# deadskull7/One-Stop-for-COVID-19-Infection-and-Lung-Segmentation-plus-Classification

Measured on AMD Instinct MI355X. Metric: CT images/sec (fwd+bwd) U-Net 512x512x1 bs16, higher is better.
Workload: dtype f32 storage / accumulate / parameters; conv products as a two-term fp16 split (3 fp16 MFMAs per multiply, ~2^-22 per product; --algo 2 = strict fp32); 1 GPU; U-Net infection seg (task1 graph T1:853-916), 512x512x1, batch 16/GPU, fp32, fwd+loss+bwd+Keras-Adam; BASELINE.json configs[1]; storage=fp32, global_batch=16, parallelism=dp1, deterministic=False, bn_fold=2

## Files before the change

include/unet_hip.h:

```cpp
#ifndef UNET_HIP_H
#define UNET_HIP_H
#include <stddef.h>
#include <stdint.h>

#ifdef __cplusplus
extern "C" {
#endif

#define UNET_ABI_VERSION 16

typedef struct unet_ctx unet_ctx;
typedef struct unet_model unet_model;
typedef uint16_t unet_bf16;
enum { UNET_DTYPE_F32 = 0, UNET_DTYPE_BF16 = 1 };

enum { UNET_OK = 0, UNET_E_ARG = -1, UNET_E_HIP = -2, UNET_E_SHAPE = -3, UNET_E_STATE = -4, UNET_E_NODEV = -5 };

enum { UNET_ALGO_AUTO = 0, UNET_ALGO_NAIVE = 1, UNET_ALGO_MFMA = 2 };

int32_t unet_abi_version(void);
int32_t unet_ctx_create(int32_t device_id, unet_ctx** out);
void unet_ctx_destroy(unet_ctx* ctx);
const char* unet_last_error(const unet_ctx* ctx);
int32_t unet_ctx_set_profiling(unet_ctx* ctx, int32_t on);
enum { UNET_OPT_RELU_BITS = 1, UNET_OPT_BN_FOLD = 2, UNET_OPT_ENC_BN_FUSED = 3, UNET_OPT_BN_CONCAT_ANALYTIC = 4, UNET_OPT_BN_FUSE_STATS = 5, UNET_OPT_DETERMINISTIC = 6,
       UNET_OPT_HEAD_FUSED = 7, UNET_OPT_SKIP_RAW = 8, UNET_OPT_POOL_SUMS_FUSED = 9, UNET_OPT_HEAD_BWD_FUSED = 10, UNET_OPT_CONV_PP = 13, UNET_OPT_ENC_TAIL_DGRAD = 14 };
int32_t unet_ctx_set_option(unet_ctx* ctx, int32_t option, int32_t value);
int32_t unet_ctx_get_option(unet_ctx* ctx, int32_t option);

enum { UNET_ACT_NONE = 0, UNET_ACT_RELU = 1, UNET_ACT_ELU = 2 };
enum { UNET_MASK_NONE = 0, UNET_MASK_RELU = 1, UNET_MASK_ELU = 2, UNET_MASK_ELU_DROP = 3, UNET_MASK_RELU_BITS = 9  };

size_t unet_conv3x3_w_ws_floats(int32_t cin, int32_t cout);
int32_t unet_conv3x3_pick_algo(int32_t algo, int32_t wd, int32_t cin, int32_t cout);
double unet_conv3x3_exec_ratio(int32_t algo, int32_t h, int32_t wd, int32_t cin, int32_t cout);
double unet_conv3x3_wgrad_exec_ratio(int32_t algo, int32_t h, int32_t wd, int32_t cin, int32_t cout);
int32_t unet_request_bn_stats(unet_ctx*, int32_t c);
int32_t unet_relu_bits_supported(int32_t algo, int32_t h, int32_t wd, int32_t cin, int32_t cout);
size_t unet_relu_bits_bytes(int32_t n, int32_t h, int32_t wd, int32_t c);
int32_t unet_request_relu_bits(unet_ctx*, void* bits);
int32_t unet_allow_k_slices(unet_ctx*);
int32_t unet_ctx_max_kernel_scratch_bytes(unet_ctx*);
int32_t unet_conv3x3_fwd(unet_ctx*, const float* x, const float* w, const float* bias, float* y,
                         int32_t n, int32_t h, int32_t wd, int32_t cin, int32_t cout,
                         int32_t act, float drop_rate, uint64_t drop_seed, int32_t algo, float* w_ws, void* stream);
int32_t unet_conv3x3_fwd_ld(unet_ctx*, const float* x, const float* w, const float* bias, float* y, int32_t ldy,
                            int32_t n, int32_t h, int32_t wd, int32_t cin, int32_t cout, int32_t act, int32_t algo, float* w_ws, void* stream);
int32_t unet_conv3x3_bwd_data(unet_ctx*, const float* dy, const float* w, const float* mask_src,
                              int32_t mask_mode, float mask_rate, uint64_t mask_seed,
                              float* dx, float* wt_ws, int32_t n, int32_t h, int32_t wd,
                              int32_t cin, int32_t cout, int32_t algo, void* stream);
int32_t unet_conv3x3_bnfold_supported(int32_t algo, int32_t h, int32_t wd, int32_t cin, int32_t cout);
size_t unet_conv3x3_bnfold_ws_floats(int32_t n, int32_t cin, int32_t cout);
int32_t unet_conv3x3_bnfold_fwd(unet_ctx*, const float* x, const float* bnp, const float* w, const float* bias, float* y, int32_t n, int32_t h,
                                int32_t wd, int32_t cin, int32_t cout, int32_t act, int32_t algo, float* ws, void* stream);
int32_t unet_conv3x3_bnfold_bwd_weights(unet_ctx*, const float* x, const float* bnp, const float* dy, const float* w, float* dw, float* db,
                                        double* bn_bwd_sums, void* gws, size_t gws_bytes, float* ws, int32_t n, int32_t h, int32_t wd,
                                        int32_t cin, int32_t cout, int32_t algo, void* stream);
int32_t unet_conv3x3_bnfold_bwd_data(unet_ctx*, const float* dy, const float* w, const float* bnp, const double* bn_bwd_sums, double count, const float* x,
                                     int32_t x_channels, int32_t mask_mode, float mask_rate, uint64_t mask_seed, float* dx, float* wt_ws, float* coef,
                                     int32_t n, int32_t h, int32_t wd, int32_t cin, int32_t cout, int32_t algo, void* stream);
int32_t unet_conv3x3_bnfold_bwd_data_enc_tail(unet_ctx*, const float* dy, const float* w, const float* bnp, const double* bn_bwd_sums, double count, const float* x, int32_t ldx,
                                              const float* enc_bnp, const double* enc_sums, double enc_count, const float* skip_k1, const float* dy_pooled, float rate,
                                              uint64_t seed, float* dx, float* wt_ws, float* coef, int32_t n, int32_t h, int32_t wd, int32_t c, int32_t algo, void* stream);
size_t unet_conv3x3_bwd_weights_ws_bytes(int32_t n, int32_t h, int32_t wd, int32_t cin, int32_t cout);
int32_t unet_conv3x3_bwd_weights(unet_ctx*, const float* x, const float* dy, float* dw, float* db,
                                 void* ws, size_t ws_bytes, int32_t n, int32_t h, int32_t wd,
                                 int32_t cin, int32_t cout, int32_t algo, void* stream);

int32_t unet_convT2x2_fwd(unet_ctx*, const float* x, const float* w, const float* bias, float* y,
                          int32_t ldy, int32_t n, int32_t h, int32_t wd, int32_t cin, int32_t cout,
                          int32_t algo, void* stream);
int32_t unet_convT2x2_bwd_data(unet_ctx*, const float* dy, int32_t lddy, const float* w,
                               const float* relu_src, float* dx, int32_t n, int32_t h, int32_t wd,
                               int32_t cin, int32_t cout, int32_t algo, void* stream);
size_t unet_convT2x2_bwd_weights_ws_bytes(int32_t n, int32_t h, int32_t wd, int32_t cin, int32_t cout);
int32_t unet_convT2x2_bwd_weights(unet_ctx*, const float* x, const float* dy, int32_t lddy,
                                  float* dw, float* db, void* ws, size_t ws_bytes, int32_t n,
                                  int32_t h, int32_t wd, int32_t cin, int32_t cout, int32_t algo,
                                  void* stream);

int32_t unet_bn_stats(unet_ctx*, const float* x, int32_t ldx, double* sums, int64_t pixels,
                      int32_t c, void* stream);
int32_t unet_bn_stats_concat(unet_ctx*, const float* x_up, int32_t ldx, const double* src_sums, double src_count, const float* src_gamma,
                             const float* src_beta, double* sums, int64_t pixels, int32_t c_up, int32_t c_skip, void* stream);
int32_t unet_bn_finalize_train(unet_ctx*, const double* sums, double count, const float* gamma,
                               const float* beta, float* moving_mean, float* moving_var,
                               float* bnp, int32_t c, void* stream);
int32_t unet_bn_finalize_infer(unet_ctx*, const float* gamma, const float* beta,
                               const float* moving_mean, const float* moving_var, float* bnp,
                               int32_t c, void* stream);
int32_t unet_bn_apply(unet_ctx*, const float* x, int32_t ldx, const float* bnp, float* y,
                      int32_t ldy, int64_t pixels, int32_t c, void* stream);
int32_t unet_bn_bwd_stats(unet_ctx*, const float* dy, int32_t lddy, const float* x, int32_t ldx,
                          const float* bnp, double* sums, int64_t pixels, int32_t c, void* stream);
int32_t unet_bn_bwd_param_grads(unet_ctx*, const double* sums, float* dgamma, float* dbeta,
                                int32_t c, void* stream);
int32_t unet_bn_bwd_apply(unet_ctx*, const float* dy, int32_t lddy, const float* x, int32_t ldx,
                          const float* bnp, const double* sums, double count, int32_t mask_mode,
                          float mask_rate, uint64_t mask_seed, float* dx, int32_t lddx, int64_t pixels,
                          int32_t c, void* stream);

int32_t unet_maxpool2x2_dropout_fwd(unet_ctx*, const float* x, int32_t ldx, float* y, int32_t n,
                                    int32_t h, int32_t wd, int32_t c, float rate, uint64_t seed,
                                    void* stream);
int32_t unet_maxpool2x2_dropout_bwd(unet_ctx*, const float* x, int32_t ldx, const float* dy,
                                    float* dx, int32_t lddx, int32_t n, int32_t h, int32_t wd,
                                    int32_t c, float rate, uint64_t seed, int32_t accumulate,
                                    void* stream);

int32_t unet_bn_apply_maxpool_dropout_fwd(unet_ctx*, const float* x, int32_t ldx, const float* bnp, float* y,
                                          int32_t ldy, float* pooled, int32_t n, int32_t h, int32_t wd,
                                          int32_t c, float rate, uint64_t seed, void* stream);
int32_t unet_maxpool2x2_dropout_bwd_bnstats(unet_ctx*, const float* y, int32_t ldy, const float* dy, float* dx,
                                            int32_t lddx, const float* gamma, const float* beta, double* sums,
                                            int32_t n, int32_t h, int32_t wd, int32_t c, float rate,
                                            uint64_t seed, void* stream);
// ... 371 lines not shown
```

one-stop-for-covid-19-infection-and-lung-segmentation-plus-classification_amd/_lib.py:

```python
from __future__ import annotations

import ctypes as C
import os

_HERE = os.path.dirname(os.path.abspath(__file__))
LIB_PATH = os.environ.get("COVIDSEG_AMD_LIB") or os.path.join(_HERE, "libunet_hip.so")
ABI_VERSION = 16
COMM_HANDLE_BYTES, COMM_MAX_WORLD, COMM_MAX_DOUBLES = 64, 8, 2048

ALGO_AUTO, ALGO_NAIVE, ALGO_MFMA = 0, 1, 2
OPTIONS = {"relu_bits": 1, "bn_fold": 2, "enc_bn_fused": 3, "bn_concat_analytic": 4, "bn_fuse_stats": 5, "deterministic": 6, "head_fused": 7, "skip_raw": 8, "pool_sums_fused": 9, "head_bwd_fused": 10, "conv_pp": 13, "enc_tail_dgrad": 14}
ARCH_UNET, ARCH_UNETPP, ARCH_CLASSIFIER = 0, 1, 2
LOSSES = {"bce_dice_loss": 0, "binary_crossentropy": 1, "dice_loss": 2, "tversky_loss": 3, "weighted_bce_dice_loss": 4}
DTYPE_F32, DTYPE_BF16 = 0, 1
ACT_NONE, ACT_RELU, ACT_ELU = 0, 1, 2
MORPH_OPS = {"dilate": 0, "erode": 1, "open": 2, "close": 3}
MORPH_MAX_ITERATIONS = 64
INTENSITY_MAX_EDGES = 63
JOINT_HIST_MAX_K, JOINT_HIST_MAX_BINS = 16, 64
SMOOTH_MAX_RADIUS = 32
PAIRS_CHUNK, PAIRS_LDS_SLOTS = 4096, 1024
PAIRS_MIN_CAPACITY, PAIRS_MAX_CAPACITY = 16, 2 ** 30
TRACK_CLS_NONE, TRACK_CLS_RESOLVED, TRACK_CLS_SHRINKAGE, TRACK_CLS_BOTH, TRACK_CLS_GROWTH, TRACK_CLS_NEW = 0, 1, 2, 3, 4, 5
TEXTURE_MAX_LEVELS, TEXTURE_MAX_DISTANCE, TEXTURE_LDS_COUNTERS = 64, 4, 8192
TEXTURE_MAX_RUN = 2 ** 15
ZONE_MAX_PARTS, ZONE_MAX_SHELLS, ZONE_MAX_BINS = 8, 4, 1024
MASK_NONE, MASK_RELU, MASK_ELU, MASK_ELU_DROP = 0, 1, 2, 3
PROG_FWD_TRAIN, PROG_BWD, PROG_FWD_INFER = 0, 1, 2
SYNC_BN_FWD, SYNC_LOSS, SYNC_BN_BWD, SYNC_GRAD_BUCKET = 0, 1, 2, 3

f32p = C.POINTER(C.c_float)
f64p = C.POINTER(C.c_double)
vp = C.c_void_p
i32, i64, u64, f32, f64, sz = C.c_int32, C.c_int64, C.c_uint64, C.c_float, C.c_double, C.c_size_t


class SyncPoint(C.Structure):
    _fields_ = [("after_op", i32), ("kind", i32), ("ptr", vp), ("count", i64), ("use_op", i32), ("reserved", i32)]


RENDER_MAX_TILES, RENDER_MAX_LAYERS = 64, 4


class RenderTile(C.Structure):
    _fields_ = [("axis", i32), ("index", i32), ("x0", i32), ("y0", i32), ("w", i32), ("h", i32)]


class RenderLayer(C.Structure):
    _fields_ = [("labels", vp), ("palette", vp), ("dtype", i32), ("palette_size", i32), ("fill_alpha", i32), ("outline_alpha", i32)]


class ZoneSpec(C.Structure):
    _fields_ = [("parts", i32 * 3), ("flip", i32 * 3), ("lo", (i32 * 3) * 2), ("extent", (i32 * 3) * 2), ("shells", i32), ("reserved", i32), ("r2", (f64 * 3) * 2)]


_PROTOS = {
    "unet_abi_version": (i32, []),
    "unet_ctx_create": (i32, [i32, C.POINTER(vp)]),
    "unet_ctx_destroy": (None, [vp]),
    "unet_last_error": (C.c_char_p, [vp]),
    "unet_ctx_set_profiling": (i32, [vp, i32]),
    "unet_ctx_set_option": (i32, [vp, i32, i32]),
    "unet_ctx_get_option": (i32, [vp, i32]),
    "unet_conv3x3_w_ws_floats": (sz, [i32, i32]),
    "unet_conv3x3_pick_algo": (i32, [i32, i32, i32, i32]),
    "unet_conv3x3_exec_ratio": (f64, [i32, i32, i32, i32, i32]),
    "unet_conv3x3_wgrad_exec_ratio": (f64, [i32, i32, i32, i32, i32]),
    "unet_request_bn_stats": (i32, [vp, i32]),
    "unet_relu_bits_supported": (i32, [i32, i32, i32, i32, i32]),
    "unet_relu_bits_bytes": (sz, [i32, i32, i32, i32]),
    "unet_request_relu_bits": (i32, [vp, vp]),
    "unet_allow_k_slices": (i32, [vp]),
    "unet_ctx_max_kernel_scratch_bytes": (i32, [vp]),
    "unet_conv3x3_fwd": (i32, [vp, vp, vp, vp, vp, i32, i32, i32, i32, i32, i32, f32, u64, i32, vp, vp]),
    "unet_conv3x3_fwd_ld": (i32, [vp, vp, vp, vp, vp, i32, i32, i32, i32, i32, i32, i32, i32, vp, vp]),
    "unet_conv3x3_bwd_data": (i32, [vp, vp, vp, vp, i32, f32, u64, vp, vp, i32, i32, i32, i32, i32, i32, vp]),
    "unet_conv3x3_bwd_weights_ws_bytes": (sz, [i32, i32, i32, i32, i32]),
    "unet_conv3x3_bwd_weights": (i32, [vp, vp, vp, vp, vp, vp, sz, i32, i32, i32, i32, i32, i32, vp]),
    "unet_convT2x2_fwd": (i32, [vp, vp, vp, vp, vp, i32, i32, i32, i32, i32, i32, i32, vp]),
    "unet_convT2x2_bwd_data": (i32, [vp, vp, i32, vp, vp, vp, i32, i32, i32, i32, i32, i32, vp]),
    "unet_convT2x2_bwd_weights_ws_bytes": (sz, [i32, i32, i32, i32, i32]),
    "unet_convT2x2_bwd_weights": (i32, [vp, vp, vp, i32, vp, vp, vp, sz, i32, i32, i32, i32, i32, i32, vp]),
    "unet_cast_f32_to_bf16": (i32, [vp, vp, vp, i64, vp]),
    "unet_cast_bf16_to_f32": (i32, [vp, vp, vp, i64, vp]),
    "unet_conv3x3_fwd_bf16": (i32, [vp, vp, vp, vp, vp, i32, i32, i32, i32, i32, i32, f32, u64, vp, vp]),
    "unet_conv3x3_first_fwd_bf16": (i32, [vp, vp, vp, vp, vp, i32, i32, i32, i32, i32, f32, u64, vp]),
    "unet_conv3x3_bwd_data_bf16": (i32, [vp, vp, vp, vp, i32, f32, u64, vp, vp, i32, i32, i32, i32, i32, vp]),
    "unet_conv3x3_bwd_weights_ws_bytes_bf16": (sz, [i32, i32, i32, i32, i32]),
    "unet_conv3x3_bwd_weights_bf16": (i32, [vp, vp, vp, vp, vp, vp, sz, i32, i32, i32, i32, i32, vp]),
    "unet_conv3x3_first_bwd_weights_bf16": (i32, [vp, vp, vp, vp, vp, vp, sz, i32, i32, i32, i32, vp]),
    "unet_convT2x2_fwd_bf16": (i32, [vp, vp, vp, vp, vp, i32, i32, i32, i32, i32, i32, vp, vp]),
    "unet_convT2x2_bwd_data_bf16": (i32, [vp, vp, i32, vp, vp, vp, i32, i32, i32, i32, i32, vp, vp]),
    "unet_convT2x2_bwd_weights_ws_bytes_bf16": (sz, [i32, i32, i32, i32, i32]),
    "unet_convT2x2_bwd_weights_bf16": (i32, [vp, vp, vp, i32, vp, vp, vp, sz, i32, i32, i32, i32, i32, vp]),
    "unet_bn_stats": (i32, [vp, vp, i32, vp, i64, i32, vp]),
    "unet_bn_stats_bf16": (i32, [vp, vp, i32, vp, i64, i32, vp]),
    "unet_conv3x3_bnfold_supported": (i32, [i32, i32, i32, i32, i32]),
    "unet_conv3x3_bnfold_ws_floats": (sz, [i32, i32, i32]),
    "unet_conv3x3_bnfold_fwd": (i32, [vp, vp, vp, vp, vp, vp, i32, i32, i32, i32, i32, i32, i32, vp, vp]),
    "unet_conv3x3_bnfold_bwd_weights": (i32, [vp, vp, vp, vp, vp, vp, vp, vp, vp, sz, vp, i32, i32, i32, i32, i32, i32, vp]),
    "unet_conv3x3_bnfold_bwd_data": (i32, [vp, vp, vp, vp, vp, f64, vp, i32, i32, f32, u64, vp, vp, vp, i32, i32, i32, i32, i32, i32, vp]),
    "unet_conv3x3_bnfold_bwd_data_enc_tail": (i32, [vp, vp, vp, vp, vp, f64, vp, i32, vp, vp, f64, vp, vp, f32, u64, vp, vp, vp, i32, i32, i32, i32, i32, vp]),
    "unet_bn_stats_concat": (i32, [vp, vp, i32, vp, f64, vp, vp, vp, i64, i32, i32, vp]),
    "unet_bn_stats_concat_bf16": (i32, [vp, vp, i32, vp, f64, vp, vp, vp, i64, i32, i32, vp]),
    "unet_bn_finalize_train": (i32, [vp, vp, f64, vp, vp, vp, vp, vp, i32, vp]),
    "unet_bn_finalize_infer": (i32, [vp, vp, vp, vp, vp, vp, i32, vp]),
    "unet_bn_apply": (i32, [vp, vp, i32, vp, vp, i32, i64, i32, vp]),
    "unet_bn_apply_bf16": (i32, [vp, vp, i32, vp, vp, i32, i64, i32, vp]),
    "unet_bn_bwd_stats": (i32, [vp, vp, i32, vp, i32, vp, vp, i64, i32, vp]),
    "unet_bn_bwd_stats_bf16": (i32, [vp, vp, i32, vp, i32, vp, vp, i64, i32, vp]),
    "unet_bn_bwd_param_grads": (i32, [vp, vp, vp, vp, i32, vp]),
    "unet_bn_bwd_apply": (i32, [vp, vp, i32, vp, i32, vp, vp, f64, i32, f32, u64, vp, i32, i64, i32, vp]),
    "unet_bn_bwd_apply_bf16": (i32, [vp, vp, i32, vp, i32, vp, vp, f64, i32, f32, u64, vp, i32, i64, i32, vp]),
    "unet_maxpool2x2_dropout_fwd": (i32, [vp, vp, i32, vp, i32, i32, i32, i32, f32, u64, vp]),
    "unet_maxpool2x2_dropout_fwd_bf16": (i32, [vp, vp, i32, vp, i32, i32, i32, i32, f32, u64, vp]),
    "unet_maxpool2x2_dropout_bwd": (i32, [vp, vp, i32, vp, vp, i32, i32, i32, i32, i32, f32, u64, i32, vp]),
    "unet_maxpool2x2_dropout_bwd_bf16": (i32, [vp, vp, i32, vp, vp, i32, i32, i32, i32, i32, f32, u64, i32, vp]),
    "unet_bn_apply_maxpool_dropout_fwd": (i32, [vp, vp, i32, vp, vp, i32, vp, i32, i32, i32, i32, f32, u64, vp]),
    "unet_bn_apply_maxpool_dropout_fwd_bf16": (i32, [vp, vp, i32, vp, vp, i32, vp, i32, i32, i32, i32, f32, u64, vp]),
    "unet_maxpool2x2_dropout_bwd_bnstats": (i32, [vp, vp, i32, vp, vp, i32, vp, vp, vp, i32, i32, i32, i32, f32, u64, vp]),
    "unet_maxpool2x2_dropout_bwd_sums": (i32, [vp, vp, vp, vp, vp, vp, i32, i32, i32, i32, f32, u64, vp]),
    "unet_maxpool2x2_dropout_bwd_sums_bf16": (i32, [vp, vp, vp, vp, vp, vp, i32, i32, i32, i32, f32, u64, vp]),
    "unet_bn_maxpool_bwd_apply_bf16": (i32, [vp, vp, i32, vp, vp, f64, vp, i32, vp, vp, i32, i32, i32, i32, i32, f32, u64, vp]),
    "unet_bn_bwd_skip_term": (i32, [vp, vp, vp, vp, vp, vp, i32, f64, vp]),
    "unet_bn_maxpool_bwd_apply": (i32, [vp, vp, i32, vp, vp, f64, vp, i32, vp, vp, i32, i32, i32, i32, i32, f32, u64, vp]),
    "unet_maxpool2x2_dropout_bwd_bnstats_bf16": (i32, [vp, vp, i32, vp, vp, i32, vp, vp, vp, i32, i32, i32, i32, f32, u64, vp]),
    "unet_head_fwd": (i32, [vp, vp, vp, vp, vp, vp, vp, i64, i32, vp]),
    "unet_head_fwd_bf16": (i32, [vp, vp, vp, vp, vp, vp, vp, i64, i32, vp]),
    "unet_loss_finalize": (i32, [vp, vp, f64, vp, vp]),
    "unet_head_bwd": (i32, [vp, vp, vp, vp, vp, vp, f64, vp, vp, vp, i64, i32, i32, vp]),
    "unet_head_bwd_bf16": (i32, [vp, vp, vp, vp, vp, vp, f64, vp, vp, vp, i64, i32, i32, vp]),
    "unet_loss_finalize_ex": (i32, [vp, vp, f64, i32, f32, f32, vp, vp]),
    "unet_head_bwd_ex": (i32, [vp, vp, vp, vp, vp, vp, f64, i32, f32, f32, vp, vp, vp, vp, i64, i32, i32, vp]),
    "unet_head_bwd_bf16_ex": (i32, [vp, vp, vp, vp, vp, vp, f64, i32, f32, f32, vp, vp, vp, vp, i64, i32, i32, vp]),
    "unet_head_fwd_ex": (i32, [vp, vp, vp, vp, vp, vp, vp, vp, i64, i32, vp]),
    "unet_head_fwd_bf16_ex": (i32, [vp, vp, vp, vp, vp, vp, vp, vp, i64, i32, vp]),
    "unet_loss_weight_map": (i32, [vp, vp, vp, i32, i32, i32, vp]),
    "unet_conv3x3_head_fwd_ex": (i32, [vp, vp, vp, vp, vp, vp, vp, vp, vp, vp, vp, vp, i32, i32, i32, i32, vp, vp]),
    "unet_adam_keras": (i32, [vp, vp, vp, vp, vp, i64, f32, f32, f32, f32, f32, vp]),
    "unet_seg_metrics_sweep": (i32, [vp, vp, vp, vp, i32, vp, i64, vp]),
    "unet_gather_samples": (i32, [vp, vp, vp, vp, i64, i64, vp]),
    "unet_augment_samples": (i32, [vp, vp, vp, vp, vp, vp, vp, i64, i32, i32, i32, vp]),
    "unet_feat_col_mean": (i32, [vp, vp, i64, i64, i64, vp, vp]),
    "unet_feat_gemm_nt_workspace": (sz, [i64, i64, i64, i32]),
    "unet_feat_gemm_nt": (i32, [vp, vp, i64, vp, vp, i64, vp, i64, i64, i64, i32, vp, i64, i32, vp, sz, vp]),
    "unet_feat_gemm_tn_workspace": (sz, [i64, i64, i64]),
    "unet_feat_gemm_tn": (i32, [vp, vp, i64, vp, i64, vp, i64, i64, i64, vp, i64, i32, vp, sz, vp]),
    "unet_kmeans_step": (i32, [vp, vp, i64, i64, i64, vp, i32, vp, vp, vp, vp, vp, vp]),
    "unet_cluster_route_workspace": (sz, [i64, i64, i32]),
    "unet_cluster_route": (i32, [vp, vp, i32, i64, i32, i32, i32, i64, vp, vp, i32, vp, i32, vp, vp, vp, vp, sz, vp]),
    "unet_conv3x3_head_supported": (i32, [vp, i32, i32, i32, i32]),
    "unet_conv3x3_head_fwd": (i32, [vp, vp, vp, vp, vp, vp, vp, vp, vp, vp, vp, i32, i32, i32, i32, vp, vp]),
    "unet_conv3x3_bwd_data_pool_sums_supported": (i32, [vp, i32, i32, i32, i32]),
    "unet_conv3x3_bwd_data_pool_sums": (i32, [vp, vp, vp, vp, vp, vp, f32, vp, vp, vp, i32, i32, i32, i32, i32, vp]),
    "unet_head_dy": (i32, [vp, vp, vp, vp, f64, vp, vp, vp, vp, vp, vp, vp, i32, i32, i32, vp]),
# ... 195 lines not shown
```

one-stop-for-covid-19-infection-and-lung-segmentation-plus-classification_amd/csrc/common.h:

```cpp
#pragma once
#include <hip/hip_runtime.h>
#include <stdint.h>
#include <stdio.h>
#include <set>
#include <string>

#include "../../include/unet_hip.h"

constexpr int UNET_BN_SLOTS = 64, UNET_BN_SLOTS_DET = 1024, UNET_BN_SLOT_DOUBLES = 2048;
struct unet_loss_sel { int32_t kind = UNET_LOSS_BCE_DICE; float alpha = 0.5f, beta = 0.5f; };
inline bool unet_loss_sel_ok(const unet_loss_sel& ls, const float* wm = nullptr, bool need_map = true) {
  if (ls.kind < UNET_LOSS_BCE_DICE || ls.kind > UNET_LOSS_WEIGHTED_BCE_DICE) return false;
  if (ls.kind == UNET_LOSS_TVERSKY && !(ls.alpha > 0.0f && ls.beta > 0.0f && ls.alpha < 1e30f && ls.beta < 1e30f)) return false;
  return !need_map || (ls.kind == UNET_LOSS_WEIGHTED_BCE_DICE) == (wm != nullptr);
}
constexpr int UNET_HEAD_SUMS = 100;
struct unet_ctx {
  int device = 0;
  int num_cu = 256;
  int profiling = 0;
  int opt_relu_bits = 1;
  int opt_bn_fold = 2;
  int opt_enc_bn_fused = 1;
  int opt_bn_concat_analytic = 1;
  int opt_bn_fuse_stats = 1;
  int opt_pool_sums_fused = 1;
  int opt_skip_raw = 1;
  int opt_head_fused = 1;
  int opt_head_bwd_fused = 1;
  int opt_enc_tail_dgrad = 1;
  int opt_conv_pp = 1;
  int opt_deterministic = 0;
  double* bn_slots = nullptr;
  int bn_nslots() const { return opt_deterministic ? UNET_BN_SLOTS_DET : UNET_BN_SLOTS; }
  void* convt_img = nullptr;
  size_t convt_img_bytes = 0;
  int k_slices_ok = 0;
  void* splitk_ws = nullptr;
  size_t splitk_ws_bytes = 0;
  int stats_req_c = 0;
  const void* stats_in_slots = nullptr;
  int stats_in_slots_c = 0;
  bool stats_in_slots_xs = false;
  unsigned long long* signs_req = nullptr;
  const void* signs_done = nullptr;
  std::set<const void*> big_lds_kernels;
  std::set<const void*> noted_kernels;
  int max_scratch_bytes = 0;
  std::string err;
};

#define UNET_FAIL(ctx, code, ...)                         \
  do {                                                    \
    char _b[512];                                         \
    snprintf(_b, sizeof(_b), __VA_ARGS__);                \
    if (ctx) (ctx)->err = _b;                             \
    return (code);                                        \
  } while (0)

#define UNET_CHECK_LAUNCH(ctx, what)                                              \
  do {                                                                            \
    hipError_t _e = hipGetLastError();                                            \
    if (_e != hipSuccess) UNET_FAIL(ctx, UNET_E_HIP, "%s: %s", what, hipGetErrorString(_e)); \
  } while (0)

#define UNET_HIP(ctx, expr)                                                       \
  do {                                                                            \
    hipError_t _e = (expr);                                                       \
    if (_e != hipSuccess) UNET_FAIL(ctx, UNET_E_HIP, "%s: %s", #expr, hipGetErrorString(_e)); \
  } while (0)

static inline int32_t unet_big_lds(unet_ctx* ctx, const void* kernel, size_t bytes, const char* what) {
  if (ctx->big_lds_kernels.count(kernel)) return UNET_OK;
  if (hipFuncSetAttribute(kernel, hipFuncAttributeMaxDynamicSharedMemorySize, (int)bytes) != hipSuccess) UNET_FAIL(ctx, UNET_E_HIP, "%s: cannot reserve %zu bytes of LDS", what, bytes);
  ctx->big_lds_kernels.insert(kernel);
  return UNET_OK;
}
static inline void unet_note_kernel(unet_ctx* ctx, const void* kernel) {
  if (ctx->noted_kernels.count(kernel)) return;
  ctx->noted_kernels.insert(kernel);
  hipFuncAttributes at;
  if (hipFuncGetAttributes(&at, kernel) == hipSuccess && (int)at.localSizeBytes > ctx->max_scratch_bytes) ctx->max_scratch_bytes = (int)at.localSizeBytes;
}
// ... 143 lines not shown
}

enum { ACT_NONE = 0, ACT_RELU = 1, ACT_ELU = 2 };
__device__ __forceinline__ float apply_act(float v, int act) {
  if (act == ACT_RELU) return fmaxf(v, 0.0f);
  if (act == ACT_ELU) return v > 0.0f ? v : expm1f(v);
  return v;
}
enum { MASK_NONE = 0, MASK_RELU = 1, MASK_ELU = 2, MASK_ELU_DROP = 3 };
enum { MASK_BIAS_TAB = 4 };
enum { MASK_BN_BWD = 5 };
enum { MASK_BN_BWD_ELU = 6, MASK_BN_BWD_ELU_DROP = 7 };
enum { MASK_BN_BWD_RELU = 8 };
enum { MASK_RELU_BITS = 9 };
enum { MASK_POOL_SUMS = 10 };
int32_t k_bn_bwd_coef(unet_ctx*, const float* bnp, const double* sums, double count, float* coef, int c, hipStream_t s);
__device__ __forceinline__ float mask_factor(float m, int mode, float ks , float rate) {
  if (mode == MASK_RELU) return m > 0.0f ? 1.0f : 0.0f;
  if (mode == MASK_ELU) return m > 0.0f ? 1.0f : m + 1.0f;
  if (mode == MASK_ELU_DROP) { const float a = m * (1.0f - rate); return ks * (a > 0.0f ? 1.0f : a + 1.0f); }
  return 1.0f;
}

size_t bn_fold_scratch_floats(int cin, int cout);
int32_t k_bn_fold_prepare(unet_ctx*, const float* w, const float* bias, const float* scale, const float* shift, int cin, int cout, float* scratch, hipStream_t s, bool want_scaled = true);
size_t wgrad_bn_fold_scratch_floats(int n, int cout);
bool wgrad_bn_fold_supported(int cout);
int32_t k_wgrad_bn_fold_fix(unet_ctx*, const float* dy, int n, int h, int wd, int cin, int cout, const float* scale, const float* shift, float* dw, const float* db, float* scratch,
                            hipStream_t s, const float* w = nullptr, const float* mean = nullptr, const float* istd = nullptr, double* bn_bwd_sums = nullptr,
                            const float* pre_s = nullptr, const float* pre_t = nullptr,
                            float* dgamma = nullptr, float* dbeta = nullptr);
int32_t k_wgrad_bn_fold_fix_bf16(unet_ctx*, const unet_bf16* dy, int n, int h, int wd, int cin, int cout, const float* scale, const float* shift, float* dw, const float* db,
                                 float* scratch, hipStream_t s, const float* w = nullptr, const float* mean = nullptr, const float* istd = nullptr, double* bn_bwd_sums = nullptr);
constexpr int UNET_PREP_MAX = 36;
bool h2_conv3x3_selected(int algo, int K, int M);
bool pp_conv3x3_selected(const unet_ctx* ctx, int K, int M, int n, int h, int wd, const float* mask, int mask_mode, int act, float rate, int ldy);
int32_t k_conv3x3_pp_fwd(unet_ctx*, const float* x, const void* wimg, const float* bias, const float* mask, int mask_mode, float* y, int ldy, int n, int h, int wd, int K, int M,
                         int act, hipStream_t s, bool vdy = false);
size_t h2_wimg_bytes(int K, int M);
int32_t k_h2_weights(unet_ctx*, const float* w, void* img, int cin, int cout, int flip, hipStream_t s, const float* cs = nullptr);
int32_t k_h2_weights_multi(unet_ctx*, const float* const* w, void* const* img, const int* cin, const int* cout, const int* flip, int count, hipStream_t s);
int32_t k_h2_weights_bound(unet_ctx*, const float* w, const float* cs, void* img, int cin, int cout, hipStream_t s);
int32_t k_h2_prep_multi(unet_ctx*, const float* const* w, const float* const* cs, void* const* img, const int* cin, const int* cout, const int* kind, int count, hipStream_t s);
size_t h2_convT_img_bytes(int cin, int cout);
int32_t k_conv3x3_h2_fwd(unet_ctx*, const float* x, const void* wimg, const float* bias, const float* mask, int mask_mode, float* y, int n, int h, int wd, int K, int M,
                         int act, float rate, uint64_t seed, hipStream_t s, int mask_climit = 1 << 30, int ldy = 0);
int32_t k_slot_fold(unet_ctx*, double* sums, int count, hipStream_t s, bool xs = false);
int32_t k_enc_tail_finish(unet_ctx*, double* sums, const double* dec_sum_dyxhat, const float* dec_invstd, const float* dec_gamma, const float* gamma, float* dgamma, float* dbeta, int c,
                          double frac, hipStream_t s);
bool h2_enc_tail_dgrad_selected(const unet_ctx* ctx, int algo, int n, int h, int wd, int C, bool force);
int32_t k_conv3x3_h2_dgrad_bn_bwd_up(unet_ctx*, const float* dy, const void* wimg, const float* coef, const float* x, float* dx, int n, int h, int wd, int C, hipStream_t s);
int32_t k_conv3x3_h2_dgrad_enc_tail(unet_ctx*, const float* dy, const void* wimg, const float* coef, const float* x, int ldx, const float* enc_bnp, const double* enc_sums, double count,
                                    const float* skip_k1, const float* dy_pooled, float* dx, int n, int h, int wd, int C, float rate, uint64_t seed, hipStream_t s);
bool h2_pool_sums_selected(const unet_ctx* ctx, int algo, int wd, int K, int M);
int32_t k_conv3x3_h2_dgrad_pool_sums(unet_ctx*, const float* dy, const void* wimg, const float* pooled, const float* gamma, const float* beta, float rate, float* dx, double* sums,
                                     int n, int h, int wd, int K, int M, hipStream_t s);
int32_t k_bn_finalize_compose(unet_ctx*, int training, const double* sums, double count, const float* gamma, const float* beta, float* mm, float* mv, float* bnp, int c,
                              const float* enc_bnp, float* comp, hipStream_t s);
int32_t k_loss_finalize(unet_ctx*, const double* loss_sums, double count, float* loss_out, float* loss_out2, hipStream_t s, unet_loss_sel ls = {});
int32_t k_cls_loss_finalize(unet_ctx*, const double* sums, double count, float* out, float* out2, hipStream_t s);
int32_t k_bn_compose(unet_ctx*, const float* bnp_dec, const float* bnp_enc, float* comp, int c, hipStream_t s);
struct h2_head_args { const float* w = nullptr; const float* b = nullptr; float* p = nullptr; const float* t = nullptr; double* slots = nullptr; float aux = 0.0f; const float* wm = nullptr; double inv_count = 0.0; };
bool h2_conv3x3_head_selected(const unet_ctx* ctx, int algo, int wd, int K, int M);
int32_t k_conv3x3_h2_head_fwd(unet_ctx*, const float* x, const void* wimg, const float* bias, float* y, const float* wh, const float* bh, float* p, const float* t,
                              int n, int h, int wd, int K, hipStream_t s, const float* wm = nullptr);
int32_t k_head_fold(unet_ctx*, double* loss_sums, double* head_sums, hipStream_t s, bool weighted = false);
int32_t k_loss_weight_map(unet_ctx*, const float* y_true, float* weight, int n, int h, int wd, hipStream_t s);
int32_t k_head_dy(unet_ctx*, const float* p, const float* t, const double* loss_sums, double count, const double* head_sums, const float* w, const unsigned long long* bits,
                  const float* y, float* dy, float* dw, float* db, int n, int h, int wd, hipStream_t s, unet_loss_sel ls = {}, const float* wm = nullptr);
int32_t k_bn_maxpool_bwd_apply_k1(unet_ctx*, const float* x, int ldx, const float* bnp, const double* sums, double count, const float* g_skip, int ldg, const float* skip_k1,
                                  const float* dy_pooled, float* dx, int lddx, int n, int h, int wd, int c, float rate, uint64_t seed, hipStream_t s);
bool h2_convT_selected(const unet_ctx* ctx, int algo, int cin, int cout);
int32_t k_convT_h2_fwd(unet_ctx*, const float* x, const float* w, const float* bias, float* y, int ldy, int n, int h, int wd, int cin, int cout, hipStream_t s, const void* prepared = nullptr);
int32_t k_convT_h2_dgrad(unet_ctx*, const float* dy, int lddy, const float* w, const float* mask, float* dx, int n, int h, int wd, int cin, int cout, hipStream_t s, int mask_bits = 0,
                         const void* prepared = nullptr);
bool h2_wgrad_selected(int algo, int cin, int cout);
bool h2_wgrad_c16_selected(int algo, int wd, int cin, int cout);
size_t h2_wgrad_c16_ws_bytes(int n, int h, int wd);
int32_t k_wgrad_c16_gather(unet_ctx*, const float* G, float* dw, float* db, hipStream_t s);
int32_t k_conv3x3_h2_wgrad_c16(unet_ctx*, const float* x, const float* dy, float* dw, float* db, void* ws, size_t ws_bytes, int n, int h, int wd, hipStream_t s);
size_t h2_wgrad_ws_bytes(int n, int h, int wd, int cin, int cout);
int32_t k_conv3x3_h2_wgrad(unet_ctx*, const float* x, const float* dy, float* dw, float* db, void* ws, size_t ws_bytes, int n, int h, int wd, int cin, int cout, hipStream_t s);
int32_t k_head_dzm(unet_ctx*, const float* p, const float* t, const double* loss_sums, double count, const double* head_sums, const unsigned long long* bits, void* dzm, float* dw,
                   float* db, int n, int h, int wd, hipStream_t s, unet_loss_sel ls = {}, const float* wm = nullptr);
bool h2_head_bwd_selected(const unet_ctx* ctx, int algo, int wd, int cin);
int32_t k_conv3x3_h2_dgrad_dzm(unet_ctx*, const void* dzm, const void* wimg, const float* mask, int mask_mode, float* dx, int n, int h, int wd, int M, hipStream_t s);
int32_t k_conv3x3_h2_wgrad_dzm(unet_ctx*, const float* x, const void* dzm, const float* w_head, float* dw, float* db, void* ws, size_t ws_bytes, int n, int h, int wd, int cin,
                               hipStream_t s);
int32_t k_conv3x3_naive_fwd(unet_ctx*, const float* x, const float* w, const float* bias, const float* mask, int mask_mode,
                            float* y, int n, int h, int wd, int cin, int cout, int act, float rate, uint64_t seed, hipStream_t s);
bool c1_relu_bits_supported(int wd, int cout);
int32_t k_conv3x3_c1_fwd_bits(unet_ctx*, const float* x, const float* w, const float* bias, float* y, unsigned long long* signs, int n, int h, int wd, int cout, hipStream_t s);
int32_t k_conv3x3_c1_fwd(unet_ctx*, const float* x, const float* w, const float* bias, float* y, int n, int h,
                         int wd, int cout, int act, float rate, uint64_t seed, hipStream_t s);
size_t c1_wgrad_ws_bytes(int cout);
int32_t k_conv3x3_c1_wgrad(unet_ctx*, const float* x, const float* dy, float* dw, float* db, void* ws, size_t ws_bytes, int n, int h,
                           int wd, int cout, hipStream_t s);
int32_t k_flip_transpose_w3x3(unet_ctx*, const float* w, float* wt, int cin, int cout, hipStream_t s);
int32_t k_conv3x3_naive_wgrad(unet_ctx*, const float* x, const float* dy, float* dw, float* db, int n, int h,
                              int wd, int cin, int cout, hipStream_t s);
int32_t k_convT_naive_fwd(unet_ctx*, const float* x, const float* w, const float* bias, float* y, int ldy, int n,
                          int h, int wd, int cin, int cout, hipStream_t s);
int32_t k_convT_naive_dgrad(unet_ctx*, const float* dy, int lddy, const float* w, const float* mask, float* dx,
                            int n, int h, int wd, int cin, int cout, hipStream_t s);
int32_t k_convT_naive_wgrad(unet_ctx*, const float* x, const float* dy, int lddy, float* dw, float* db, int n,
                            int h, int wd, int cin, int cout, hipStream_t s);
// ... 47 lines not shown
```

one-stop-for-covid-19-infection-and-lung-segmentation-plus-classification_amd/csrc/kernels_conv_h2.hip:

```cpp
#include <stdlib.h>

#include <algorithm>

#include "common.h"

#ifndef H2_EXPERIMENT
#define H2_EXPERIMENT 0
#endif

#if H2_EXPERIMENT == 5
__device__ unsigned long long h2_trace[16384 * 16];
#define H2_STAMP(i) do { if (tid == 0 && blockIdx.x < 16384) h2_trace[blockIdx.x * 16 + (i)] = __builtin_readcyclecounter(); } while (0)
extern "C" int32_t unet_debug_h2_trace(unsigned long long* host, int n) {
  return hipMemcpyFromSymbol(host, HIP_SYMBOL(h2_trace), (size_t)n * 8) == hipSuccess ? 0 : 1;
}
#else
#define H2_STAMP(i) do { } while (0)
#endif
namespace {

typedef _Float16 f16x8 __attribute__((ext_vector_type(8)));
typedef _Float16 f16x2 __attribute__((ext_vector_type(2)));
typedef unet_f32x16 f32x16;
constexpr int H2_HEADER = 256;
// ... 48 lines not shown
#pragma unroll
  for (int o = 32; o >= 1; o >>= 1) mx = fmaxf(mx, __shfl_xor(mx, o));
  if (p.cs_bound) {
    float mc = 0.f;
    for (int i = threadIdx.x & 63; i < p.cs_mod; i += 64) mc = fmaxf(mc, fabsf(p.cs[i]));
#pragma unroll
    for (int o = 32; o >= 1; o >>= 1) mc = fmaxf(mc, __shfl_xor(mc, o));
    mx *= mc;
  }
  const int eb = (int)((__float_as_uint(mx) >> 23) & 0xFF);
  int e = eb >= 11 ? scale_exp_for(eb) : 0;
  e = min(max(e, -100), 100);
  const float sc = pow2f(e);
  if (blockIdx.x == 0 && threadIdx.x == 0) { hdr[0] = pow2f(-e); hdr[1] = sc; }
  unet_bf16* const img = p.img + H2_HEADER / 2;
  for (long long el = (long long)blockIdx.x * 256 + threadIdx.x; el < p.total; el += (long long)gridDim.x * 256) {
    long long r = el;
    const int m = (int)(r & 31); r >>= 5;
    const int half = (int)(r & 1); r >>= 1;
    const int nb = (int)(r % NB); r /= NB;
    const int tap = (int)(r % T); r /= T;
    const int ks = (int)(r % KS); r /= KS;
    const int chunk = (int)(r % nchunks); const int g = (int)(r / nchunks);
    const long long k0 = ((long long)chunk * KS + ks) * 16 + half * 8;
    const long long mm = ((long long)g * NB + nb) * 32 + cperm(m);
    const float* src = p.w + (long long)(p.flip ? T - 1 - tap : tap) * p.tap_stride + k0 * p.sk + mm * p.sm;
    unsigned hh[4], ml[4];
#pragma unroll
    for (int j = 0; j < 4; ++j) {
      float a = mm < M ? src[(2 * j) * p.sk] * sc : 0.0f, b = mm < M ? src[(2 * j + 1) * p.sk] * sc : 0.0f;
      if (p.cs) { a *= p.cs[k0 + 2 * j]; b *= p.cs[k0 + 2 * j + 1]; }
      split2(a, b, hh[j], ml[j]);
    }
    const long long base = ((((((long long)g * nchunks + chunk) * KS + ks) * T + tap) * NB + nb) * 2 * 2 + half) * 32 + m;
    *reinterpret_cast<uint4*>(img + (base + 0 * 64) * 8) = make_uint4(hh[0], hh[1], hh[2], hh[3]);
    *reinterpret_cast<uint4*>(img + (base + 1 * 64) * 8) = make_uint4(ml[0], ml[1], ml[2], ml[3]);
  }
}

__device__ __forceinline__ f16x8 lds_frag(const char* p) { return *reinterpret_cast<const f16x8*>(p); }
__device__ __forceinline__ int out_cell(int p, int c) { return p * 128 + ((c ^ (p & 7)) << 4); }

template <int MODE, int NB, int RW, bool GEN, int WPS, int EPI = 0, bool SPLITK = false>
__global__ __launch_bounds__(256, WPS) void conv_h2_kernel(const float* __restrict__ x, int ldx, const unet_bf16* __restrict__ wimg_hdr, const float* __restrict__ bias,
                                                           const float* __restrict__ mask, float* __restrict__ y, int ldy, int N, int H, int W, int K, int M, int act,
                                                           int mask_mode, float rate, unsigned long long seed, int tiles_x, int tiles_y, int groups,
                                                           int total_blocks, double* __restrict__ stats, int stats_c, unsigned long long* __restrict__ signs,
                                                           int mask_climit, h2_head_args hd, int img_nb, int xs, int kcps, long long y_split, int g0, int gtot, int ldm, int c_off) {
  constexpr bool HEAD = EPI == 1 || EPI == 4, WHEAD = EPI == 4, POOLS = EPI == 2;
  constexpr bool VDY = EPI == 3;
  constexpr bool ETAIL = EPI == 5;
  static_assert(!ETAIL || (MODE == 0 && RW == 2 && !GEN && !SPLITK), "the encoder-tail epilogue rides on the 8-row conv3x3 data-gradient launches");
  if (ETAIL) { mask_mode = MASK_BN_BWD; act = ACT_NONE; stats = nullptr; signs = nullptr; }
  static_assert(!VDY || (MODE == 0 && NB == 1 && RW == 2 && !GEN), "the virtual head gradient feeds the 32-channel data-gradient launch");
  static_assert(!HEAD || (MODE == 0 && NB == 1 && RW == 2 && !GEN), "the fused head rides on the 32-channel forward kernel");
  static_assert(!POOLS || (MODE == 0 && !GEN), "the pooled sums ride on a plain conv3x3 data-gradient launch");
  static_assert(!SPLITK || (MODE == 0 && EPI == 0 && !GEN), "K slices: plain conv3x3 launches");
  if (POOLS) { mask_mode = MASK_POOL_SUMS; act = ACT_NONE; signs = nullptr; }
  if (HEAD) { mask_mode = MASK_NONE; act = ACT_RELU; stats = nullptr; }
  constexpr int T = MODE == 0 ? 9 : 1, KS = MODE == 0 ? 1 : 2;
  constexpr int TH = 4 * RW;
  constexpr int PR = MODE == 0 ? TH + 2 : TH, PWD = MODE == 0 ? 34 : 32, NPIX = PR * PWD;
  constexpr int HS = NPIX * 16 + (MODE == 0 ? 0 : 64);
  constexpr int PLANE = KS * 2 * HS;
  constexpr int IN_BYTES = 2 * PLANE, W_BYTES = KS * T * NB * 2 * 2 * 32 * 16;
  constexpr int PPIECES = KS * NPIX * 4, WPIECES = W_BYTES / 16;
  constexpr int PL = (PPIECES + 255) / 256, WL = (WPIECES + 255) / 256;
  constexpr int OUT_PS = 128;
  constexpr bool WPAD = NB != 1 || MODE != 0;
  constexpr int W_LDS = WPAD ? WL * 256 * 16 : W_BYTES;
  extern __shared__ __attribute__((aligned(16))) char smem[];
  char* const s_in = smem; char* const s_w = smem + IN_BYTES;
  float* const s_amax = reinterpret_cast<float*>(smem + IN_BYTES + W_LDS);
  float* const s_bias = s_amax + 4;

  const int tid = threadIdx.x, lane = tid & 63, l31 = lane & 31, hi = lane >> 5;
  const int wave = __builtin_amdgcn_readfirstlane(tid >> 6);
  const int per = gridDim.x >> 3;
  const int wi = (blockIdx.x & 7) * per + (blockIdx.x >> 3);
  if (wi >= total_blocks) return;
  const int g = g0 + wi % groups; int t = wi / groups;
  const int tx = t % tiles_x; t /= tiles_x;
  const int ty = t % tiles_y; const int n = t / tiles_y;
  const int x0 = tx * 32, y0 = ty * TH;
  const int HI = MODE == 2 ? 2 * H : H, WI = MODE == 2 ? 2 * W : W;
  const int nchunks = K / (16 * KS);
  const int cbeg = SPLITK ? (int)blockIdx.y * kcps : 0, cend = SPLITK ? min(cbeg + kcps, nchunks) : nchunks;
  if (SPLITK) y += (long long)blockIdx.y * y_split;
  const unet_bf16* const wimg = wimg_hdr + H2_HEADER / 2;
  const float w_unscale = *reinterpret_cast<const float*>(wimg_hdr);

  f32x16 acc[RW][NB];
#pragma unroll
  for (int i = 0; i < RW; ++i)
#pragma unroll
    for (int j = 0; j < NB; ++j)
#pragma unroll
      for (int r = 0; r < 16; ++r) acc[i][j][r] = 0.0f;

  const __amdgpu_buffer_rsrc_t rs_x = make_rsrc(x + (long long)n * HI * WI * ldx, (long long)HI * WI * ldx * 4);
  const __amdgpu_buffer_rsrc_t rs_w = __builtin_amdgcn_make_buffer_rsrc(const_cast<unet_bf16*>(wimg), 0, (int)((long long)gtot * nchunks * W_BYTES), 0x00020000);
  int poff[PL];
#pragma unroll
  for (int k = 0; k < PL; ++k) {
    const int idx = tid + k * 256;
    const int q = idx & 3, pp = idx >> 2, ks = pp / NPIX, pix = pp - ks * NPIX;
// ... 375 lines not shown
        gp[q * 4] = g4.x; gp[q * 4 + 1] = g4.y; gp[q * 4 + 2] = g4.z; gp[q * 4 + 3] = g4.w;
      }
#pragma unroll
      for (int r = 0; r < RW; ++r)
#pragma unroll
        for (int j = 0; j < 4; ++j) *reinterpret_cast<float4*>(s_x + r * 4096 + out_cell(j * 8 + (lane >> 3), lane & 7)) = mpre[nb][r][j];
#pragma unroll
      for (int q = 0; q < 4; ++q) {
        const int cc = nb * 32 + hi * 16 + q * 4;
        const float4 xa4 = *reinterpret_cast<const float4*>(s_x + out_cell(l31, hi * 4 + q)), xb4 = *reinterpret_cast<const float4*>(s_x + 4096 + out_cell(l31, hi * 4 + q));
        const float4 c0 = *reinterpret_cast<const float4*>(s_bias + cc), ck = *reinterpret_cast<const float4*>(s_bias + NB * 32 + cc), c2 = *reinterpret_cast<const float4*>(s_bias + 2 * NB * 32 + cc);
        const float4 sc4 = *reinterpret_cast<const float4*>(s_co + cc), sh4 = *reinterpret_cast<const float4*>(s_co + NB * 32 + cc), mn4 = *reinterpret_cast<const float4*>(s_co + 2 * NB * 32 + cc);
        const float4 is4 = *reinterpret_cast<const float4*>(s_co + 3 * NB * 32 + cc), k14 = *reinterpret_cast<const float4*>(s_co + 4 * NB * 32 + cc), k24 = *reinterpret_cast<const float4*>(s_co + 5 * NB * 32 + cc);
        const float xa[4] = {xa4.x, xa4.y, xa4.z, xa4.w}, xb[4] = {xb4.x, xb4.y, xb4.z, xb4.w};
        const float K0[4] = {c0.x, c0.y, c0.z, c0.w}, kk[4] = {ck.x, ck.y, ck.z, ck.w}, K2[4] = {c2.x, c2.y, c2.z, c2.w}, sc[4] = {sc4.x, sc4.y, sc4.z, sc4.w}, sh[4] = {sh4.x, sh4.y, sh4.z, sh4.w};
        const float mean[4] = {mn4.x, mn4.y, mn4.z, mn4.w}, istd[4] = {is4.x, is4.y, is4.z, is4.w}, k1[4] = {k14.x, k14.y, k14.z, k14.w}, k2[4] = {k24.x, k24.y, k24.z, k24.w};
#pragma unroll
        for (int c = 0; c < 4; ++c) {
          const int i = q * 4 + c;
          const float gsa = fmaf(K0[c], acc[0][nb][i] * unscale, K2[c]), gsb = fmaf(K0[c], acc[1][nb][i] * unscale, K2[c]);
          const float ya = fmaf(xa[c], sc[c], sh[c]), yb = fmaf(xb[c], sc[c], sh[c]);
          const float pa = __int_as_float(__builtin_amdgcn_update_dpp(0, __float_as_int(ya), 0xB1, 0xF, 0xF, true));
          const float pb = __int_as_float(__builtin_amdgcn_update_dpp(0, __float_as_int(yb), 0xB1, 0xF, 0xF, true));
          const int kmax = argmax4(odd ? pa : ya, odd ? ya : pa, odd ? pb : yb, odd ? yb : pb);
          const float ta = fmaf(kk[c], ya, gsa) + (kmax == odd ? gp[i] : 0.f);
          const float tb = fmaf(kk[c], yb, gsb) + (kmax == 2 + odd ? gp[i] : 0.f);
          acc[0][nb][i] = xa[c] > 0.f ? sc[c] * (ta - k1[c] - (xa[c] - mean[c]) * istd[c] * k2[c]) : 0.f;
          acc[1][nb][i] = xb[c] > 0.f ? sc[c] * (tb - k1[c] - (xb[c] - mean[c]) * istd[c] * k2[c]) : 0.f;
        }
      }
#pragma unroll
      for (int r = 0; r < RW; ++r) {
        const int py = py0 + r;
#pragma unroll
        for (int q = 0; q < 4; ++q)
          *reinterpret_cast<float4*>(s_x + out_cell(l31, hi * 4 + q)) = make_float4(acc[r][nb][q * 4], acc[r][nb][q * 4 + 1], acc[r][nb][q * 4 + 2], acc[r][nb][q * 4 + 3]);
        float4 t4s[4];
#pragma unroll
        for (int j = 0; j < 4; ++j) t4s[j] = *reinterpret_cast<const float4*>(s_x + out_cell(j * 8 + (lane >> 3), lane & 7));
        asm volatile("" :: "v"(t4s[0].x), "v"(t4s[1].x), "v"(t4s[2].x), "v"(t4s[3].x));
#pragma unroll
        for (int j = 0; j < 4; ++j) {
          const int pxj = x0 + j * 8 + (lane >> 3), cj = lane & 7;
          if (pxj < W && mb0 + cj * 4 < M) {
            float* const q = y + (((long long)n * H + py) * W + pxj) * ldy + (mb0 - c_off) + cj * 4;
            __builtin_nontemporal_store(t4s[j].x, q); __builtin_nontemporal_store(t4s[j].y, q + 1); __builtin_nontemporal_store(t4s[j].z, q + 2); __builtin_nontemporal_store(t4s[j].w, q + 3);
          }
        }
      }
    }
    H2_STAMP(8);
    return;
  }
#pragma unroll
  for (int nb = 0; nb < NB; ++nb) {
    const int mb0 = (g * NB + nb) * 32, mb = mb0 + hi * 16;
    if (mb0 >= M) continue;
    int ab = 0, oc = mb;
    if (MODE == 1) { const int ct = M >> 2; ab = mb / ct; oc = mb - ab * ct; }
    float bv[16];
#pragma unroll
    for (int q = 0; q < 4; ++q) {
      const float4 b4 = *reinterpret_cast<const float4*>(s_bias + nb * 32 + hi * 16 + q * 4);
      bv[q * 4] = b4.x; bv[q * 4 + 1] = b4.y; bv[q * 4 + 2] = b4.z; bv[q * 4 + 3] = b4.w;
    }
    float4 st1 = make_float4(0.f, 0.f, 0.f, 0.f), st2 = st1;
#pragma unroll
    for (int r = 0; r < RW; ++r) {
      const int py = y0 + wave * RW + r;
      if (py >= H) continue;
      const bool live = px_ < W && mb < M;
      long long o;
      if (MODE == 1) o = (((long long)n * 2 * H + 2 * py + (ab >> 1)) * (2 * W) + 2 * px_ + (ab & 1)) * ldy + oc;
      else o = (((long long)n * H + py) * W + px_) * ldy + mb;
      float v[16], mv[16], a[16];
#pragma unroll
      for (int i = 0; i < 16; ++i) a[i] = acc[r][nb][i] * unscale;
      if (mask_mode == MASK_RELU_BITS) {
        float4 w01, w23;
        if (MPF) { w01 = mpre[MPF ? nb : 0][MPF ? r : 0][0]; w23 = mpre[MPF ? nb : 0][MPF ? r : 0][1]; }
        else {
          const bool ok = py < H && x0 + (l31 & ~7) < W;
          const unsigned long long* p = reinterpret_cast<const unsigned long long*>(mask) + ((((long long)n * H + py) * (W >> 3) + (x0 >> 3) + (l31 >> 3)) * (M >> 5) + (g * NB + nb)) * 4;
          w01 = ok ? *reinterpret_cast<const float4*>(p) : make_float4(0.f, 0.f, 0.f, 0.f);
          w23 = ok ? *reinterpret_cast<const float4*>(p + 2) : make_float4(0.f, 0.f, 0.f, 0.f);
        }
        const bool up = (l31 & 4) != 0;
        const unsigned d[4] = {__float_as_uint(up ? w01.y : w01.x), __float_as_uint(up ? w01.w : w01.z), __float_as_uint(up ? w23.y : w23.x), __float_as_uint(up ? w23.w : w23.z)};
        const int sh = (l31 & 3) * 8 + hi * 4;
#pragma unroll
        for (int q = 0; q < 4; ++q)
#pragma unroll
          for (int k = 0; k < 4; ++k) mv[q * 4 + k] = ((d[k] >> (sh + q)) & 1u) ? 1.0f : 0.0f;
      } else if (want_m && !POOLS) {
        if (MPF) {
#pragma unroll
          for (int j = 0; j < 4; ++j) *reinterpret_cast<float4*>(s_out + out_cell(j * 8 + (lane >> 3), lane & 7)) = mpre[MPF ? nb : 0][MPF ? r : 0][j];
        }
#pragma unroll
        for (int q = 0; q < 4; ++q) {
          float4 m4;
          if (MPF) m4 = *reinterpret_cast<const float4*>(s_out + out_cell(l31, hi * 4 + q));
          else m4 = (live && mb0 < mask_climit) ? *reinterpret_cast<const float4*>(mask + (((long long)n * H + py) * W + px_) * ldm + (mb - c_off) + q * 4) : make_float4(0.f, 0.f, 0.f, 0.f);
          mv[q * 4] = m4.x; mv[q * 4 + 1] = m4.y; mv[q * 4 + 2] = m4.z; mv[q * 4 + 3] = m4.w;
        }
      }
      if (mask_mode >= MASK_BN_BWD && mask_mode <= MASK_BN_BWD_RELU) {
#pragma unroll
        for (int q = 0; q < 4; ++q) {
          const float4 k1 = *reinterpret_cast<const float4*>(s_bias + (NB + nb) * 32 + hi * 16 + q * 4), k2 = *reinterpret_cast<const float4*>(s_bias + (2 * NB + nb) * 32 + hi * 16 + q * 4);
          v[q * 4] = fmaf(bv[q * 4], a[q * 4], fmaf(k1.x, mv[q * 4], k2.x));
          v[q * 4 + 1] = fmaf(bv[q * 4 + 1], a[q * 4 + 1], fmaf(k1.y, mv[q * 4 + 1], k2.y));
          v[q * 4 + 2] = fmaf(bv[q * 4 + 2], a[q * 4 + 2], fmaf(k1.z, mv[q * 4 + 2], k2.z));
          v[q * 4 + 3] = fmaf(bv[q * 4 + 3], a[q * 4 + 3], fmaf(k1.w, mv[q * 4 + 3], k2.w));
        }
        if (mask_mode == MASK_BN_BWD_RELU) {
#pragma unroll
          for (int i = 0; i < 16; ++i) v[i] = mv[i] > 0.f ? v[i] : 0.f;
        }
      } else if (mask_mode == MASK_BIAS_TAB && (py == 0 || py == H - 1 || px_ == 0 || px_ == W - 1)) {
        const int cls = (((py == 0) | ((py == H - 1) << 1)) << 2) | ((px_ == 0) | ((px_ == W - 1) << 1));
        const float* tb = mask + (long long)cls * M + mb;
#pragma unroll
        for (int q = 0; q < 4; ++q) {
          const float4 b4 = *reinterpret_cast<const float4*>(tb + q * 4);
          v[q * 4] = a[q * 4] + b4.x; v[q * 4 + 1] = a[q * 4 + 1] + b4.y; v[q * 4 + 2] = a[q * 4 + 2] + b4.z; v[q * 4 + 3] = a[q * 4 + 3] + b4.w;
        }
      } else {
#pragma unroll
        for (int i = 0; i < 16; ++i) v[i] = a[i] + bv[i];
      }
      if (!GEN) {
        if (act == ACT_RELU) {
#pragma unroll
          for (int i = 0; i < 16; ++i) v[i] = fmaxf(v[i], 0.f);
        }
        if (mask_mode == MASK_RELU || mask_mode == MASK_RELU_BITS) {
#pragma unroll
          for (int i = 0; i < 16; ++i) v[i] = mv[i] > 0.f ? v[i] : 0.f;
        }
      } else {
#pragma unroll
        for (int i = 0; i < 16; ++i) v[i] = apply_act(v[i], act);
        if (mask_mode >= MASK_BN_BWD && mask_mode <= MASK_BN_BWD_RELU) {
          if (mask_mode == MASK_BN_BWD_ELU || mask_mode == MASK_BN_BWD_ELU_DROP) {
            const int mm = mask_mode == MASK_BN_BWD_ELU_DROP ? MASK_ELU_DROP : MASK_ELU;
#pragma unroll
            for (int q = 0; q < 4; ++q) {
              float4 ks4 = make_float4(1.f, 1.f, 1.f, 1.f);
              if (mm == MASK_ELU_DROP) ks4 = keep_scale((o >> 2) + q, rate, seed);
              v[q * 4] *= mask_factor(mv[q * 4], mm, ks4.x, rate); v[q * 4 + 1] *= mask_factor(mv[q * 4 + 1], mm, ks4.y, rate);
              v[q * 4 + 2] *= mask_factor(mv[q * 4 + 2], mm, ks4.z, rate); v[q * 4 + 3] *= mask_factor(mv[q * 4 + 3], mm, ks4.w, rate);
            }
          }
        } else if (mask_mode == MASK_NONE || mask_mode == MASK_BIAS_TAB) {
          if (rate > 0.0f) {
#pragma unroll
            for (int q = 0; q < 4; ++q) {
              const float4 ks4 = keep_scale((o >> 2) + q, rate, seed);
              v[q * 4] *= ks4.x; v[q * 4 + 1] *= ks4.y; v[q * 4 + 2] *= ks4.z; v[q * 4 + 3] *= ks4.w;
            }
          }
        } else {
#pragma unroll
          for (int q = 0; q < 4; ++q) {
            float4 ks4 = make_float4(1.f, 1.f, 1.f, 1.f);
            if (mask_mode == MASK_ELU_DROP) ks4 = keep_scale((o >> 2) + q, rate, seed);
            v[q * 4] *= mask_factor(mv[q * 4], mask_mode, ks4.x, rate); v[q * 4 + 1] *= mask_factor(mv[q * 4 + 1], mask_mode, ks4.y, rate);
            v[q * 4 + 2] *= mask_factor(mv[q * 4 + 2], mask_mode, ks4.z, rate); v[q * 4 + 3] *= mask_factor(mv[q * 4 + 3], mask_mode, ks4.w, rate);
          }
        }
      }
#pragma unroll
      for (int q = 0; q < 4; ++q)
        *reinterpret_cast<float4*>(s_out + out_cell(l31, hi * 4 + q)) = make_float4(v[q * 4], v[q * 4 + 1], v[q * 4 + 2], v[q * 4 + 3]);
      float4 t4s[4];
      if (!GEN) {
#pragma unroll
        for (int j = 0; j < 4; ++j) t4s[j] = *reinterpret_cast<const float4*>(s_out + out_cell(j * 8 + (lane >> 3), lane & 7));
        asm volatile("" :: "v"(t4s[0].x), "v"(t4s[1].x), "v"(t4s[2].x), "v"(t4s[3].x));
      }
#pragma unroll
      for (int j = 0; j < 4; ++j) {
        const int pj = j * 8 + (lane >> 3), cj = lane & 7, pxj = x0 + pj;
        const float4 t4 = GEN ? *reinterpret_cast<const float4*>(s_out + out_cell(pj, cj)) : t4s[j];
        long long oj;
        if (MODE == 1) oj = (((long long)n * 2 * H + 2 * py + (ab >> 1)) * (2 * W) + 2 * pxj + (ab & 1)) * ldy + (oc - hi * 16);
        else oj = (((long long)n * H + py) * W + pxj) * ldy + (mb - hi * 16);
        if (MODE == 0 && !GEN && signs) {
          const unsigned long long bb[4] = {__builtin_amdgcn_ballot_w64(t4.x > 0.f), __builtin_amdgcn_ballot_w64(t4.y > 0.f), __builtin_amdgcn_ballot_w64(t4.z > 0.f), __builtin_amdgcn_ballot_w64(t4.w > 0.f)};
          int slo = 0, shi = 0;
          unet_writelane(slo, (unsigned)bb[0], 0); unet_writelane(shi, (unsigned)(bb[0] >> 32), 0); unet_writelane(slo, (unsigned)bb[1], 1); unet_writelane(shi, (unsigned)(bb[1] >> 32), 1);
          unet_writelane(slo, (unsigned)bb[2], 2); unet_writelane(shi, (unsigned)(bb[2] >> 32), 2); unet_writelane(slo, (unsigned)bb[3], 3); unet_writelane(shi, (unsigned)(bb[3] >> 32), 3);
          if (lane < 4 && x0 + j * 8 < W)
            signs[((((long long)n * H + py) * (W >> 3) + (x0 >> 3) + j) * (M >> 5) + (g * NB + nb)) * 4 + lane] = ((unsigned long long)(unsigned)shi << 32) | (unsigned)slo;
        }
        if (pxj < W && mb0 + cj * 4 < M) {
          {
            float* const q = y + oj + cj * 4;
            __builtin_nontemporal_store(t4.x, q); __builtin_nontemporal_store(t4.y, q + 1); __builtin_nontemporal_store(t4.z, q + 2); __builtin_nontemporal_store(t4.w, q + 3);
          }
          if (POOLS) {
            const float4 pv = MPF ? mpre[MPF ? nb : 0][MPF ? r : 0][j] : *reinterpret_cast<const float4*>(mask + oj + cj * 4);
            const float4 ig = *reinterpret_cast<const float4*>(s_bias + (NB + nb) * 32 + cj * 4), be = *reinterpret_cast<const float4*>(s_bias + (2 * NB + nb) * 32 + cj * 4);
            const float unkeep = 1.0f - hd.aux, inv = 1.0f / unkeep;
            const bool drop = hd.aux > 0.0f;
            const float kx = drop && __float_as_uint(pv.x) == 0x80000000u ? 0.f : inv, ky = drop && __float_as_uint(pv.y) == 0x80000000u ? 0.f : inv;
            const float kz = drop && __float_as_uint(pv.z) == 0x80000000u ? 0.f : inv, kw = drop && __float_as_uint(pv.w) == 0x80000000u ? 0.f : inv;
            const float gx = t4.x * kx, gy = t4.y * ky, gz = t4.z * kz, gw = t4.w * kw;
            st1.x += gx; st1.y += gy; st1.z += gz; st1.w += gw;
            st2.x = fmaf(gx, (pv.x * unkeep - be.x) * ig.x, st2.x); st2.y = fmaf(gy, (pv.y * unkeep - be.y) * ig.y, st2.y);
            st2.z = fmaf(gz, (pv.z * unkeep - be.z) * ig.z, st2.z); st2.w = fmaf(gw, (pv.w * unkeep - be.w) * ig.w, st2.w);
          } else
          if (MODE != 2 && stats) {
            st1.x += t4.x; st1.y += t4.y; st1.z += t4.z; st1.w += t4.w;
            st2.x = fmaf(t4.x, t4.x, st2.x); st2.y = fmaf(t4.y, t4.y, st2.y); st2.z = fmaf(t4.z, t4.z, st2.z); st2.w = fmaf(t4.w, t4.w, st2.w);
          }
        }
      }
    }
    if (MODE != 2 && stats) {
      float sv[8] = {st1.x, st1.y, st1.z, st1.w, st2.x, st2.y, st2.z, st2.w};
#pragma unroll
      for (int i = 0; i < 8; ++i) {
        sv[i] += __shfl_xor(sv[i], 8); sv[i] += __shfl_xor(sv[i], 16); sv[i] += __shfl_xor(sv[i], 32);
      }
      if (lane < 8) {
#pragma unroll
        for (int i = 0; i < 4; ++i) { s_stat[((wave * NB + nb) * 2 + 0) * 32 + lane * 4 + i] = sv[i]; s_stat[((wave * NB + nb) * 2 + 1) * 32 + lane * 4 + i] = sv[4 + i]; }
      }
    }
  }
  H2_STAMP(12);
  if (MODE != 2 && stats) {
    __syncthreads();
    if (tid < NB * 64) {
      const int nb = tid >> 6, kind = (tid >> 5) & 1, c32 = tid & 31;
      const int mb = (g * NB + nb) * 32;
      if (mb + c32 < M) {
        float t = 0.f;
#pragma unroll
        for (int wv = 0; wv < 4; ++wv) t += s_stat[((wv * NB + nb) * 2 + kind) * 32 + c32];
        int ch = mb + c32;
        if (MODE == 1) ch = ch % (M >> 2);
        double* const row = stats + (size_t)(blockIdx.x % UNET_BN_SLOTS) * UNET_BN_SLOT_DOUBLES;
        if (xs) xsum_add(row, (kind ? stats_c : 0) + ch, t); else atomicAdd(row + (kind ? stats_c : 0) + ch, (double)t);
      }
    }
  }
  H2_STAMP(8);
#if H2_EXPERIMENT == 5
  if (tid == 0 && blockIdx.x < 16384) { unsigned hw; asm volatile("s_getreg_b32 %0, hwreg(HW_REG_HW_ID)" : "=s"(hw)); h2_trace[blockIdx.x * 16 + 9] = hw;
    unsigned xcc; asm volatile("s_getreg_b32 %0, hwreg(HW_REG_XCC_ID)" : "=s"(xcc)); h2_trace[blockIdx.x * 16 + 10] = xcc; }
#endif
}

template <int MODE, int NB, int RW, int WPS, int EPI = 0>
int32_t launch_h2(unet_ctx* ctx, const float* x, int ldx, const unet_bf16* wimg, const float* bias, const float* mask, int mask_mode, float* y, int ldy, int n, int h, int wd,
                  int K, int M, int act, float rate, unsigned long long seed, hipStream_t s, int mask_climit = 1 << 30, h2_head_args hd = h2_head_args(), int img_nb = 0,
                  int splits = 1, int g0 = 0, int ng = 0, int ldm = 0, int c_off = 0) {
  constexpr int T = MODE == 0 ? 9 : 1, KS = MODE == 0 ? 1 : 2;
  if (img_nb == 0) img_nb = NB;
  if (img_nb != NB && !(MODE != 2 && NB == 1 && (img_nb == 2 || img_nb == 4) && (M % (32 * img_nb)) == 0 && (EPI == 0 || EPI == 5))) UNET_FAIL(ctx, UNET_E_ARG, "conv h2: image of %d blocks per group on a %d-block launch", img_nb, NB);
  constexpr int TH = 4 * RW;
  constexpr int NPIX = MODE == 0 ? (TH + 2) * 34 : TH * 32;
  constexpr size_t smem = (size_t)2 * KS * 2 * (NPIX * 16 + (MODE == 0 ? 0 : 64)) + (NB != 1 || MODE != 0 ? (size_t)((KS * T * NB * 2 * 2 * 32 + 255) / 256) * 256 * 16 : (size_t)KS * T * NB * 2 * 2 * 32 * 16) + 16 + 3 * NB * 32 * 4;
  if (!mask) mask_mode = MASK_NONE;
  const int tiles_x = (wd + 31) / 32, tiles_y = (h + TH - 1) / TH, gtot = (M + 32 * NB - 1) / (32 * NB), groups = ng ? ng : gtot;
  if (g0 < 0 || groups < 1 || g0 + groups > gtot || (splits > 1 && groups != gtot)) UNET_FAIL(ctx, UNET_E_ARG, "conv h2: channel groups [%d, %d) of %d", g0, g0 + groups, gtot);
  if (ldm == 0) ldm = ldy;
  const long long total = (long long)tiles_x * tiles_y * n * groups;
  if (total >= (1LL << 28)) UNET_FAIL(ctx, UNET_E_SHAPE, "conv h2: too many tiles");
  const unsigned grid = (unsigned)(8 * ((total + 7) / 8));
  const bool gen = MODE == 0 && (act == ACT_ELU || rate > 0.0f || mask_mode == MASK_ELU || mask_mode == MASK_ELU_DROP || mask_mode == MASK_BN_BWD_ELU || mask_mode == MASK_BN_BWD_ELU_DROP);
  double* stats = nullptr; int stats_c = 0;
  if (MODE != 2 && ctx->stats_req_c > 0) {
    const int c = ctx->stats_req_c; ctx->stats_req_c = 0;
    const int xw = ctx->opt_deterministic ? UNET_XW : 1;
    if ((mask_mode == MASK_NONE || mask_mode == MASK_BIAS_TAB) && 2 * c * xw <= UNET_BN_SLOT_DOUBLES && c == (MODE == 1 ? M / 4 : M) && ctx->bn_slots) {
      stats = ctx->bn_slots; stats_c = c; ctx->stats_in_slots = y; ctx->stats_in_slots_c = c; ctx->stats_in_slots_xs = ctx->opt_deterministic != 0;
    }
  }
  if (mask_mode == MASK_POOL_SUMS) {
    if (MODE != 0 || !ctx->bn_slots || 2 * M * (ctx->opt_deterministic ? UNET_XW : 1) > UNET_BN_SLOT_DOUBLES) UNET_FAIL(ctx, UNET_E_ARG, "conv h2: the pooled-sums epilogue is a conv3x3 data-gradient launch (M = %d)", M);
    stats = ctx->bn_slots; stats_c = M;
  }
  if (mask_mode == MASK_RELU_BITS && ((M & 31) || (wd & 7))) UNET_FAIL(ctx, UNET_E_SHAPE, "conv h2: the bit mask needs M %% 32 == 0 and W %% 8 == 0 (M=%d W=%d)", M, wd);
  unsigned long long* signs = nullptr;
  if (MODE == 0 && ctx->signs_req) {
    unsigned long long* q = ctx->signs_req; ctx->signs_req = nullptr;
    if (act == ACT_RELU && rate == 0.0f && (mask_mode == MASK_NONE || mask_mode == MASK_BIAS_TAB) && !(M & 31) && !(wd & 7)) { signs = q; ctx->signs_done = q; }
  }
  const int nchunks_ = K / (16 * KS), kcps = (nchunks_ + splits - 1) / splits;
  auto go = [&](auto kern) -> int32_t {
    if (smem > 65536) UNET_BIG_LDS(ctx, kern, smem, "conv_h2");
    unet_note_kernel(ctx, reinterpret_cast<const void*>(kern));
    hipLaunchKernelGGL(kern, dim3(grid, (unsigned)((nchunks_ + kcps - 1) / kcps)), dim3(256), smem, s, x, ldx, wimg, bias, mask, y, ldy, n, h, wd, K, M, act, mask_mode, rate, seed, tiles_x,
                       tiles_y, groups, (int)total, stats, stats_c, signs, mask_climit, hd, img_nb, ctx->opt_deterministic ? 1 : 0, kcps, (long long)n * h * wd * ldy, g0, gtot, ldm, c_off);
    return UNET_OK;
  };
  int32_t r;
  if (splits > 1) {
    if constexpr (MODE == 0 && EPI == 0 && NB == 1 && WPS == 4) {
      if (gen || stats || signs || mask_mode != MASK_NONE || bias || act != ACT_NONE || rate != 0.0f) UNET_FAIL(ctx, UNET_E_ARG, "conv h2: K slices go with a plain partial-sum launch");
      r = go(conv_h2_kernel<MODE, NB, RW, false, WPS, EPI, true>);
      if (r) return r;
      UNET_CHECK_LAUNCH(ctx, "conv_h2 (K slices)");
      return UNET_OK;
    } else UNET_FAIL(ctx, UNET_E_ARG, "conv h2: K slices exist for the one-block conv3x3 launches");
  }
  if (EPI == 1 || EPI == 4) {
    if (gen || mask_mode != MASK_NONE || act != ACT_RELU || M != 32 || stats) UNET_FAIL(ctx, UNET_E_ARG, "conv h2 + head: a plain 32-channel ReLU forward launch only");
    r = go(conv_h2_kernel<MODE, NB, RW, false, WPS, EPI>);
  } else if (EPI == 2) {
    if (gen || mask_mode != MASK_POOL_SUMS || act != ACT_NONE) UNET_FAIL(ctx, UNET_E_ARG, "conv h2 + pooled sums: a plain data-gradient launch only");
    r = go(conv_h2_kernel<MODE, NB, RW, false, WPS, EPI>);
  } else if (EPI == 5) {
    if (!mask || !bias || !hd.w || !hd.b || !hd.slots || act != ACT_NONE || (h & 1) || (wd & 1) || rate < 0.0f || rate >= 1.0f) UNET_FAIL(ctx, UNET_E_ARG, "conv h2 + encoder tail: a plain data-gradient launch over an even image only");
    r = go(conv_h2_kernel<MODE, NB, RW, false, WPS, EPI>);
  } else if (EPI == 3) {
    if (gen || K != 32 || ldx != 2 || act != ACT_NONE || mask_mode == MASK_POOL_SUMS) UNET_FAIL(ctx, UNET_E_ARG, "conv h2 behind the head's {dz, mask} stream: a plain 32-channel data-gradient launch only");
    r = go(conv_h2_kernel<MODE, NB, RW, false, WPS, EPI>);
  } else if (mask_mode == MASK_POOL_SUMS) { UNET_FAIL(ctx, UNET_E_ARG, "conv h2: MASK_POOL_SUMS goes with its own kernel instance");
  } else if (gen) r = go(conv_h2_kernel<MODE, NB, RW, (MODE == 0), WPS>); else r = go(conv_h2_kernel<MODE, NB, RW, false, WPS>);
  if (r) return r;
  UNET_CHECK_LAUNCH(ctx, "conv_h2");
  return UNET_OK;
}

__global__ __launch_bounds__(256) void h2_splitk_finish_kernel(const float* __restrict__ part, int splits, long long stride, const float* __restrict__ bias, int tab, int act,
                                                               float* __restrict__ y, int ldy, int H, int W, int M, long long total4) {
  const long long i = (long long)blockIdx.x * 256 + threadIdx.x;
  if (i >= total4) return;
  const int m4 = M >> 2, c4 = (int)(i % m4);
  const long long pix = i / m4;
  float4 a = *reinterpret_cast<const float4*>(part + i * 4);
  for (int k = 1; k < splits; ++k) {
    const float4 b = *reinterpret_cast<const float4*>(part + (long long)k * stride + i * 4);
    a.x += b.x; a.y += b.y; a.z += b.z; a.w += b.w;
  }
  if (bias) {
    int cls = 0;
    if (tab) { const int px = (int)(pix % W), py = (int)((pix / W) % H); cls = (((py == 0) | ((py == H - 1) << 1)) << 2) | ((px == 0) | ((px == W - 1) << 1)); }
    const float4 b = *reinterpret_cast<const float4*>(bias + (long long)cls * M + c4 * 4);
    a.x += b.x; a.y += b.y; a.z += b.z; a.w += b.w;
  }
  if (act == ACT_RELU) { a.x = fmaxf(a.x, 0.f); a.y = fmaxf(a.y, 0.f); a.z = fmaxf(a.z, 0.f); a.w = fmaxf(a.w, 0.f); }
  *reinterpret_cast<float4*>(y + pix * ldy + c4 * 4) = a;
}

}

static int h2_nb(int M) { return (M % 64) == 0 ? 2 : 1; }

bool h2_conv3x3_selected(int algo, int K, int M) { return algo == UNET_ALGO_AUTO && K >= 16 && (K % 16) == 0 && M >= 16 && (M % 16) == 0; }

size_t h2_wimg_bytes(int K, int M) { return (size_t)H2_HEADER + (size_t)36 * K * ((M + 31) / 32 * 32); }

static int h2_nb_convT_fwd() { return 4; }
static int h2_nb_convT_dgrad(int cin) { return (cin % 128) == 0 ? 4 : (cin % 64) == 0 ? 2 : 1; }

static void h2_fill_prep(h2_prep* p, const float* w, const float* cs, void* img, int cin, int cout, int kind) {
  p->w = w; p->cs = cs; p->img = static_cast<unet_bf16*>(img); p->flip = 0; p->cs_div = 4; p->cs_mod = 1; p->max_only = kind == 4; p->cs_bound = 0;
  if (kind == 4) kind = 0;
  int K, M;
  if (kind <= 1) {
    const int flip = kind;
    K = flip ? cout : cin; M = flip ? cin : cout;
    p->T = 9; p->KS = 1; p->nb = h2_nb(M); p->nchunks = K / 16; p->flip = flip;
    p->tap_stride = (long long)cin * cout; p->sk = flip ? 1 : cout; p->sm = flip ? cout : 1;
    p->nw4 = 9LL * cin * cout / 4;
// ... 79 lines not shown
    if (plain && ctx->splitk_ws && nchunks >= 16 && 2 * wgs < 3 * ctx->num_cu && (inb == 1 || small8 || t8 * ((M + 63) / 64) < 2 * ctx->num_cu) && (M % 32) == 0) {
      const int splits = std::min(4, nchunks / 4);
      const size_t slab = (size_t)n * h * wd * M;
      if (splits >= 2 && (size_t)splits * slab * sizeof(float) <= ctx->splitk_ws_bytes) {
        float* part = static_cast<float*>(ctx->splitk_ws);
        int32_t r;
        if (small8) r = launch_h2<0, 1, 1, 4>(ctx, x, K, img, nullptr, nullptr, MASK_NONE, part, M, n, h, wd, K, M, ACT_NONE, 0.0f, 0, s, 1 << 30, h2_head_args(), inb, splits);
        else r = launch_h2<0, 1, 2, 4>(ctx, x, K, img, nullptr, nullptr, MASK_NONE, part, M, n, h, wd, K, M, ACT_NONE, 0.0f, 0, s, 1 << 30, h2_head_args(), inb, splits);
        if (r) return r;
        const long long total4 = (long long)slab / 4;
        hipLaunchKernelGGL(h2_splitk_finish_kernel, dim3((unsigned)((total4 + 255) / 256)), dim3(256), 0, s, part, splits, (long long)slab, bias, mask && mask_mode == MASK_BIAS_TAB ? 1 : 0, act,
                           y, ldy, h, wd, M, total4);
        UNET_CHECK_LAUNCH(ctx, "conv_h2 (K slices: finish)");
        return UNET_OK;
      }
    }
  }
  if (t8 * ((M + 31) / 32) < ctx->num_cu) return launch_h2<0, 1, 1, 4>(ctx, x, K, img, bias, mask, mask_mode, y, ldy, n, h, wd, K, M, act, rate, seed, s, mask_climit, h2_head_args(), inb);
  if (inb == 1) return launch_h2<0, 1, 2, 4>(ctx, x, K, img, bias, mask, mask_mode, y, ldy, n, h, wd, K, M, act, rate, seed, s, mask_climit);
  if (t8 * ((M + 63) / 64) < 2 * ctx->num_cu) return launch_h2<0, 1, 2, 4>(ctx, x, K, img, bias, mask, mask_mode, y, ldy, n, h, wd, K, M, act, rate, seed, s, mask_climit, h2_head_args(), 2);
  const long long wgs16 = (long long)((wd + 31) / 32) * ((h + 15) / 16) * n * ((M + 63) / 64);
  if (h <= 128 && wgs16 >= 512) return launch_h2<0, 2, 4, 2>(ctx, x, K, img, bias, mask, mask_mode, y, ldy, n, h, wd, K, M, act, rate, seed, s, mask_climit);
  return launch_h2<0, 2, 2, 2>(ctx, x, K, img, bias, mask, mask_mode, y, ldy, n, h, wd, K, M, act, rate, seed, s, mask_climit);
}

static long long h2_half_wgs(int n, int h, int wd, int C, bool up, int* slots_per_cu) {
  const long long tx = (wd + 31) / 32;
  if (C % 64) { *slots_per_cu = 4; return tx * ((h + 7) / 8) * n * (C / 32); }
  *slots_per_cu = 2;
  const long long wgs16 = tx * ((h + 15) / 16) * n * (C / 64);
  if (up && h <= 128 && wgs16 >= 512) return wgs16;
  return tx * ((h + 7) / 8) * n * (C / 64);
}
bool h2_enc_tail_dgrad_selected(const unet_ctx* ctx, int algo, int n, int h, int wd, int C, bool force) {
  if (!ctx || C < 32 || (C % 32) || (h & 1) || (wd & 1) || !h2_conv3x3_selected(algo, C, 2 * C) || (long long)h * wd * 2 * C * 4 >= (1LL << 30)) return false;
  if (force) return true;
  if (C % 64 == 0 && h <= 128 && (long long)((wd + 31) / 32) * ((h + 15) / 16) * n * (2 * C / 64) >= 512) return false;
  for (int up = 0; up < 2; ++up) {
    int spc; const long long wgs = h2_half_wgs(n, h, wd, C, up != 0, &spc);
    if (wgs < 2LL * spc * ctx->num_cu) return false;
  }
  return true;
}
int32_t k_conv3x3_h2_dgrad_bn_bwd_up(unet_ctx* ctx, const float* dy, const void* wimg, const float* coef, const float* x, float* dx, int n, int h, int wd, int C, hipStream_t s) {
  if (!dy || !wimg || !coef || !x || !dx || C < 32 || (C % 32)) UNET_FAIL(ctx, UNET_E_ARG, "conv3x3 dgrad, up half: bad args (C = %d)", C);
  if ((long long)h * wd * 2 * C * 4 >= (1LL << 30)) UNET_FAIL(ctx, UNET_E_SHAPE, "conv3x3 h2: one image must stay below 1 GiB (32-bit buffer offsets)");
  const unet_bf16* img = static_cast<const unet_bf16*>(wimg);
  const int M = 2 * C;
  if (C % 64) return launch_h2<0, 1, 2, 4>(ctx, dy, C, img, coef, x, MASK_BN_BWD, dx, M, n, h, wd, C, M, ACT_NONE, 0.0f, 0, s, 1 << 30, h2_head_args(), 2, 1, 0, C / 32);
  if (h <= 128 && (long long)((wd + 31) / 32) * ((h + 15) / 16) * n * (C / 64) >= 512)
    return launch_h2<0, 2, 4, 2>(ctx, dy, C, img, coef, x, MASK_BN_BWD, dx, M, n, h, wd, C, M, ACT_NONE, 0.0f, 0, s, 1 << 30, h2_head_args(), 0, 1, 0, C / 64);
  return launch_h2<0, 2, 2, 2>(ctx, dy, C, img, coef, x, MASK_BN_BWD, dx, M, n, h, wd, C, M, ACT_NONE, 0.0f, 0, s, 1 << 30, h2_head_args(), 0, 1, 0, C / 64);
}
int32_t k_conv3x3_h2_dgrad_enc_tail(unet_ctx* ctx, const float* dy, const void* wimg, const float* coef, const float* x, int ldx, const float* enc_bnp, const double* enc_sums, double count,
                                    const float* skip_k1, const float* dy_pooled, float* dx, int n, int h, int wd, int C, float rate, uint64_t seed, hipStream_t s) {
  if (!dy || !wimg || !coef || !x || !enc_bnp || !enc_sums || !dy_pooled || !dx || C < 32 || (C % 32) || ldx < C || (ldx & 3) || (h & 1) || (wd & 1) || !(count >= 1) || rate < 0.f || rate >= 1.f)
    UNET_FAIL(ctx, UNET_E_ARG, "conv3x3 dgrad + encoder tail: bad args (C = %d, h = %d, w = %d)", C, h, wd);
  if ((long long)h * wd * std::max(2 * C, ldx) * 4 >= (1LL << 30)) UNET_FAIL(ctx, UNET_E_SHAPE, "conv3x3 h2: one image must stay below 1 GiB (32-bit buffer offsets)");
  h2_head_args hd; hd.w = enc_bnp; hd.b = dy_pooled; hd.wm = skip_k1; hd.slots = const_cast<double*>(enc_sums); hd.inv_count = 1.0 / count;
  const unet_bf16* img = static_cast<const unet_bf16*>(wimg);
  const int M = 2 * C;
  if (C % 64) return launch_h2<0, 1, 2, 4, 5>(ctx, dy, C, img, coef, x, MASK_BN_BWD, dx, C, n, h, wd, C, M, ACT_NONE, rate, seed, s, 1 << 30, hd, 2, 1, C / 32, C / 32, ldx, C);
  return launch_h2<0, 2, 2, 2, 5>(ctx, dy, C, img, coef, x, MASK_BN_BWD, dx, C, n, h, wd, C, M, ACT_NONE, rate, seed, s, 1 << 30, hd, 0, 1, C / 64, C / 64, ldx, C);
}

bool h2_pool_sums_selected(const unet_ctx* ctx, int algo, int wd, int K, int M) {
  (void)wd;
  return ctx && ctx->opt_pool_sums_fused && ctx->bn_slots && h2_conv3x3_selected(algo, K, M) && (M % 32) == 0 && 2 * M * (ctx->opt_deterministic ? UNET_XW : 1) <= UNET_BN_SLOT_DOUBLES;
}
int32_t k_conv3x3_h2_dgrad_pool_sums(unet_ctx* ctx, const float* dy, const void* wimg, const float* pooled, const float* gamma, const float* beta, float rate, float* dx, double* sums,
                                     int n, int h, int wd, int K, int M, hipStream_t s) {
  if (!dy || !wimg || !pooled || !gamma || !beta || !dx || rate < 0.f || rate >= 1.f) UNET_FAIL(ctx, UNET_E_ARG, "conv3x3 dgrad + pooled sums: bad args");
  if ((long long)h * wd * std::max(K, M) * 4 >= (1LL << 30)) UNET_FAIL(ctx, UNET_E_SHAPE, "conv3x3 h2: one image must stay below 1 GiB (32-bit buffer offsets)");
  h2_head_args hd; hd.w = gamma; hd.b = beta; hd.aux = rate;
  const unet_bf16* img = static_cast<const unet_bf16*>(wimg);
  int32_t r;
  const long long wgs16 = (long long)((wd + 31) / 32) * ((h + 15) / 16) * n * ((M + 63) / 64);
  if (h2_nb(M) == 1) r = launch_h2<0, 1, 2, 4, 2>(ctx, dy, K, img, nullptr, pooled, MASK_POOL_SUMS, dx, M, n, h, wd, K, M, ACT_NONE, 0.0f, 0, s, 1 << 30, hd);
  else if (h <= 128 && wgs16 >= 512) r = launch_h2<0, 2, 4, 2, 2>(ctx, dy, K, img, nullptr, pooled, MASK_POOL_SUMS, dx, M, n, h, wd, K, M, ACT_NONE, 0.0f, 0, s, 1 << 30, hd);
  else r = launch_h2<0, 2, 2, 2, 2>(ctx, dy, K, img, nullptr, pooled, MASK_POOL_SUMS, dx, M, n, h, wd, K, M, ACT_NONE, 0.0f, 0, s, 1 << 30, hd);
  if (r || !sums) return r;
  return k_slot_fold(ctx, sums, 2 * M, s, ctx->opt_deterministic != 0);
}

bool h2_conv3x3_head_selected(const unet_ctx* ctx, int algo, int wd, int K, int M) {
  return ctx && ctx->opt_head_fused && ctx->bn_slots && h2_conv3x3_selected(algo, K, M) && M == 32 && (wd & 7) == 0;
}
int32_t k_conv3x3_h2_head_fwd(unet_ctx* ctx, const float* x, const void* wimg, const float* bias, float* y, const float* wh, const float* bh, float* p, const float* t,
                              int n, int h, int wd, int K, hipStream_t s, const float* wm) {
  if (K < 16 || (K % 16) || !wh || !bh || !p || (wm && !t)) UNET_FAIL(ctx, UNET_E_ARG, "conv3x3 h2 + head: bad args");
  if ((long long)h * wd * std::max(K, 32) * 4 >= (1LL << 30)) UNET_FAIL(ctx, UNET_E_SHAPE, "conv3x3 h2: one image must stay below 1 GiB (32-bit buffer offsets)");
  h2_head_args hd; hd.w = wh; hd.b = bh; hd.p = p; hd.t = t; hd.slots = ctx->bn_slots; hd.wm = wm;
  if (wm) return launch_h2<0, 1, 2, 4, 4>(ctx, x, K, static_cast<const unet_bf16*>(wimg), bias, nullptr, MASK_NONE, y, 32, n, h, wd, K, 32, ACT_RELU, 0.0f, 0, s, 1 << 30, hd);
  return launch_h2<0, 1, 2, 4, 1>(ctx, x, K, static_cast<const unet_bf16*>(wimg), bias, nullptr, MASK_NONE, y, 32, n, h, wd, K, 32, ACT_RELU, 0.0f, 0, s, 1 << 30, hd);
}

bool h2_convT_selected(const unet_ctx* ctx, int algo, int cin, int cout) {
  return algo == UNET_ALGO_AUTO && ctx && ctx->convt_img && cin >= 32 && (cin % 32) == 0 && cout >= 32 && (cout % 32) == 0 &&
         (size_t)H2_HEADER + (size_t)16 * cin * cout <= ctx->convt_img_bytes;
}

size_t h2_convT_img_bytes(int cin, int cout) { return (size_t)H2_HEADER + (size_t)16 * cin * cout; }

int32_t k_convT_h2_fwd(unet_ctx* ctx, const float* x, const float* w, const float* bias, float* y, int ldy, int n, int h, int wd, int cin, int cout, hipStream_t s, const void* prepared) {
  if (!prepared) {
    const float* ws[1] = {w}; void* is[1] = {ctx->convt_img}; const int kind = 2;
// ... 26 lines not shown
```

one-stop-for-covid-19-infection-and-lung-segmentation-plus-classification_amd/csrc/model.hip:

```cpp
#include <algorithm>
#include <functional>
#include <map>
#include <set>
#include <string>
#include <vector>

#include "common.h"

extern "C" {

int32_t unet_abi_version(void) { return UNET_ABI_VERSION; }

int32_t unet_ctx_create(int32_t device_id, unet_ctx** out) {
  if (!out) return UNET_E_ARG;
  *out = nullptr;
  int ndev = 0;
  if (hipGetDeviceCount(&ndev) != hipSuccess || ndev <= 0 || device_id < 0 || device_id >= ndev) return UNET_E_NODEV;
  hipDeviceProp_t prop;
  if (hipGetDeviceProperties(&prop, device_id) != hipSuccess) return UNET_E_NODEV;
  if (std::string(prop.gcnArchName).rfind("gfx950", 0) != 0) return UNET_E_NODEV;
  unet_ctx* c = new unet_ctx();
  c->device = device_id;
  c->num_cu = prop.multiProcessorCount;
  const size_t sb = sizeof(double) * UNET_BN_SLOTS_DET * UNET_BN_SLOT_DOUBLES;
  int prev = 0;
  (void)hipGetDevice(&prev);
  if (hipSetDevice(device_id) != hipSuccess || hipMalloc(reinterpret_cast<void**>(&c->bn_slots), sb) != hipSuccess ||
      hipMemset(c->bn_slots, 0, sb) != hipSuccess) { (void)hipSetDevice(prev); delete c; return UNET_E_HIP; }
  c->convt_img_bytes = (size_t)8 << 20;
  if (hipMalloc(&c->convt_img, c->convt_img_bytes) != hipSuccess) { c->convt_img = nullptr; c->convt_img_bytes = 0; }
  c->splitk_ws_bytes = (size_t)32 << 20;
  if (hipMalloc(&c->splitk_ws, c->splitk_ws_bytes) != hipSuccess) { c->splitk_ws = nullptr; c->splitk_ws_bytes = 0; }
  (void)hipSetDevice(prev);
  *out = c;
  return UNET_OK;
}

void unet_ctx_destroy(unet_ctx* ctx) {
  if (ctx && ctx->bn_slots) (void)hipFree(ctx->bn_slots);
  if (ctx && ctx->convt_img) (void)hipFree(ctx->convt_img);
  if (ctx && ctx->splitk_ws) (void)hipFree(ctx->splitk_ws);
  delete ctx;
}
const char* unet_last_error(const unet_ctx* ctx) { return ctx ? ctx->err.c_str() : "null ctx"; }
int32_t unet_ctx_set_profiling(unet_ctx* ctx, int32_t on) { if (!ctx) return UNET_E_ARG; ctx->profiling = on; return UNET_OK; }

static int* ctx_option(unet_ctx* ctx, int32_t option) {
  switch (option) {
    case UNET_OPT_RELU_BITS: return &ctx->opt_relu_bits;
    case UNET_OPT_BN_FOLD: return &ctx->opt_bn_fold;
    case UNET_OPT_ENC_BN_FUSED: return &ctx->opt_enc_bn_fused;
    case UNET_OPT_BN_CONCAT_ANALYTIC: return &ctx->opt_bn_concat_analytic;
    case UNET_OPT_BN_FUSE_STATS: return &ctx->opt_bn_fuse_stats;
    case UNET_OPT_DETERMINISTIC: return &ctx->opt_deterministic;
    case UNET_OPT_HEAD_FUSED: return &ctx->opt_head_fused;
    case UNET_OPT_SKIP_RAW: return &ctx->opt_skip_raw;
    case UNET_OPT_POOL_SUMS_FUSED: return &ctx->opt_pool_sums_fused;
    case UNET_OPT_HEAD_BWD_FUSED: return &ctx->opt_head_bwd_fused;
    case UNET_OPT_CONV_PP: return &ctx->opt_conv_pp;
    case UNET_OPT_ENC_TAIL_DGRAD: return &ctx->opt_enc_tail_dgrad;
    default: return nullptr;
  }
}
int32_t unet_ctx_set_option(unet_ctx* ctx, int32_t option, int32_t value) {
  if (!ctx) return UNET_E_ARG;
  int* p = ctx_option(ctx, option);
  const int hi = option == UNET_OPT_BN_FOLD ? 3 : (option == UNET_OPT_CONV_PP || option == UNET_OPT_ENC_TAIL_DGRAD) ? 2 : 1;
  if (!p || value < 0 || value > hi) UNET_FAIL(ctx, UNET_E_ARG, "ctx_set_option: option %d value %d", option, value);
  *p = value;
  return UNET_OK;
}
int32_t unet_ctx_get_option(unet_ctx* ctx, int32_t option) {
  if (!ctx) return UNET_E_ARG;
  const int* p = ctx_option(ctx, option);
  if (!p) UNET_FAIL(ctx, UNET_E_ARG, "ctx_get_option: unknown option %d", option);
  return *p;
}

}

static bool use_mfma(int algo, int cin, int cout) {
  if (algo == UNET_ALGO_NAIVE) return false;
  return mfma_conv3x3_supported(cin, cout);
}
static bool use_h2(int algo, int cin, int cout, const void* uws) { return uws && h2_conv3x3_selected(algo, cin, cout); }

static int32_t conv3x3_fwd_dispatch(unet_ctx* ctx, const float* x, const float* w, const float* bias, const float* mask, int mask_mode,
                                    float* y, int n, int h, int wd, int cin, int cout, int act, float rate, uint64_t seed, int algo,
                                    hipStream_t s, float* uws = nullptr, int flip = 0, const float* prepared = nullptr, int ldy = 0) {
  if (ldy && ldy != cout && !(use_h2(algo, cin, cout, uws) && prepared)) UNET_FAIL(ctx, UNET_E_STATE, "conv3x3: a strided output (ldy %d) exists on the h2 kernels with a prepared image only", ldy);
  if (use_h2(algo, cin, cout, uws)) {
    if (prepared) return k_conv3x3_h2_fwd(ctx, x, prepared, bias, mask, mask_mode, y, n, h, wd, cin, cout, act, rate, seed, s, 1 << 30, ldy);
    int32_t r = flip ? k_h2_weights(ctx, w, uws, cout, cin, 1, s) : k_h2_weights(ctx, w, uws, cin, cout, 0, s);
    if (r) return r;
    return k_conv3x3_h2_fwd(ctx, x, uws, bias, mask, mask_mode, y, n, h, wd, cin, cout, act, rate, seed, s);
  }
  if (mask_mode >= MASK_BIAS_TAB) UNET_FAIL(ctx, UNET_E_STATE, "conv3x3: the folded-BatchNorm / bit-mask epilogues exist on the h2 kernels only (cin=%d cout=%d algo=%d)", cin, cout, algo);
  if (flip) {
    if (!uws) UNET_FAIL(ctx, UNET_E_ARG, "conv3x3 data gradient: needs the weight scratch");
    int32_t r = k_flip_transpose_w3x3(ctx, w, uws, cout, cin, s);
    if (r) return r;
    w = uws;
  }
  if (use_mfma(algo, cin, cout)) return k_conv3x3_mfma_fwd(ctx, x, w, bias, mask, mask_mode, y, n, h, wd, cin, cout, act, rate, seed, s);
  if (cin == 1 && !mask && algo != UNET_ALGO_NAIVE && (cout % 4) == 0 && 256 % (cout / 4) == 0) {
    if (ctx->signs_req && act == ACT_RELU && rate == 0.0f && c1_relu_bits_supported(wd, cout)) {
      unsigned long long* q = ctx->signs_req; ctx->signs_req = nullptr;
      int32_t r = k_conv3x3_c1_fwd_bits(ctx, x, w, bias, y, q, n, h, wd, cout, s);
      if (!r) ctx->signs_done = q;
      return r;
    }
    return k_conv3x3_c1_fwd(ctx, x, w, bias, y, n, h, wd, cout, act, rate, seed, s);
  }
  return k_conv3x3_naive_fwd(ctx, x, w, bias, mask, mask_mode, y, n, h, wd, cin, cout, act, rate, seed, s);
}

static int32_t conv3x3_wgrad_dispatch(unet_ctx* ctx, const float* x, const float* dy, float* dw, float* db, void* ws,
                                      size_t ws_bytes, int n, int h, int wd, int cin, int cout, int algo, hipStream_t s) {
  if (algo != UNET_ALGO_NAIVE && mfma_wgrad_supported(cin, cout) && ws && ws_bytes >= mfma_wgrad_ws_bytes(n, h, wd, cin, cout)) {
    if (h2_wgrad_c16_selected(algo, wd, cin, cout) && ws_bytes >= h2_wgrad_c16_ws_bytes(n, h, wd))
// ... 178 lines not shown
  if (!unet_conv3x3_bnfold_supported(algo, h, wd, cin, cout)) UNET_FAIL(ctx, UNET_E_SHAPE, "conv3x3_bnfold_fwd: no folded form for h=%d w=%d cin=%d cout=%d (unet_conv3x3_bnfold_supported)", h, wd, cin, cout);
  hipStream_t s = as_stream(stream);
  float* u = ws + bn_fold_scratch_floats(cin, cout);
  int32_t r = k_bn_fold_prepare(ctx, w, bias, bnp, bnp + cin, cin, cout, ws, s, false);
  if (r) return r;
  r = k_h2_weights(ctx, w, u, cin, cout, 0, s, bnp);
  if (r) return r;
  const float* tab = ws + (size_t)9 * cin * cout;
  r = k_conv3x3_h2_fwd(ctx, x, u, tab, tab, MASK_BIAS_TAB, y, n, h, wd, cin, cout, act, 0.0f, 0, s);
  ctx->k_slices_ok = 0;
  return r;
}
int32_t unet_conv3x3_bnfold_bwd_weights(unet_ctx* ctx, const float* x, const float* bnp, const float* dy, const float* w, float* dw, float* db, double* bn_bwd_sums, void* gws,
                                        size_t gws_bytes, float* ws, int32_t n, int32_t h, int32_t wd, int32_t cin, int32_t cout, int32_t algo, void* stream) {
  if (!ctx || !x || !bnp || !dy || !dw || !db || !ws || n < 1 || h < 1 || wd < 1 || cin < 1) UNET_FAIL(ctx, UNET_E_ARG, "conv3x3_bnfold_bwd_weights: bad args");
  if (!wgrad_bn_fold_supported(cout)) UNET_FAIL(ctx, UNET_E_SHAPE, "conv3x3_bnfold_bwd_weights: cout=%d (needs a divisor of 256)", cout);
  hipStream_t s = as_stream(stream);
  int32_t r = conv3x3_wgrad_dispatch(ctx, x, dy, dw, db, gws, gws_bytes, n, h, wd, cin, cout, algo, s);
  if (r) return r;
  if (bn_bwd_sums && !w) UNET_FAIL(ctx, UNET_E_ARG, "conv3x3_bnfold_bwd_weights: bn_bwd_sums needs the kernel w");
  return k_wgrad_bn_fold_fix(ctx, dy, n, h, wd, cin, cout, bnp, bnp + cin, dw, db, ws + bn_fold_scratch_floats(cin, cout) + unet_conv3x3_w_ws_floats(cin, cout), s,
                             bn_bwd_sums ? w : nullptr, bn_bwd_sums ? bnp + 2 * cin : nullptr, bn_bwd_sums ? bnp + 3 * cin : nullptr, bn_bwd_sums);
}
int32_t unet_conv3x3_bnfold_bwd_data(unet_ctx* ctx, const float* dy, const float* w, const float* bnp, const double* bn_bwd_sums, double count, const float* x, int32_t x_channels,
                                     int32_t mask_mode, float mask_rate, uint64_t mask_seed, float* dx, float* wt_ws, float* coef, int32_t n, int32_t h, int32_t wd, int32_t cin,
                                     int32_t cout, int32_t algo, void* stream) {
  if (!ctx || !dy || !w || !bnp || !bn_bwd_sums || !x || !dx || !wt_ws || !coef || n < 1 || !(count >= 1) || mask_mode < MASK_NONE || mask_mode > MASK_ELU_DROP || !(mask_rate >= 0) ||
      mask_rate >= 1)
    UNET_FAIL(ctx, UNET_E_ARG, "conv3x3_bnfold_bwd_data: bad args");
  if (!unet_conv3x3_bnfold_supported(algo, h, wd, cin, cout))
    UNET_FAIL(ctx, UNET_E_SHAPE, "conv3x3_bnfold_bwd_data: no folded form for h=%d w=%d cin=%d cout=%d (unet_conv3x3_bnfold_supported)", h, wd, cin, cout);
  if (x_channels != cin && (x_channels < 32 || x_channels > cin || (x_channels % 32) || mask_mode != MASK_NONE))
    UNET_FAIL(ctx, UNET_E_ARG, "conv3x3_bnfold_bwd_data: x_channels %d (cin = %d, or a multiple of 32 below it with UNET_MASK_NONE)", x_channels, cin);
  static const int modes[4] = {MASK_BN_BWD, MASK_BN_BWD_RELU, MASK_BN_BWD_ELU, MASK_BN_BWD_ELU_DROP};
  hipStream_t s = as_stream(stream);
  int32_t r = k_bn_bwd_coef(ctx, bnp, bn_bwd_sums, count, coef, cin, s);
  if (!r) r = k_h2_weights(ctx, w, wt_ws, cin, cout, 1, s);
  const bool drop = mask_mode == MASK_ELU_DROP;
  if (!r) r = k_conv3x3_h2_fwd(ctx, dy, wt_ws, coef, x, modes[mask_mode], dx, n, h, wd, cout, cin, ACT_NONE, drop ? mask_rate : 0.0f, drop ? mask_seed : 0, s, x_channels < cin ? x_channels : 1 << 30);
  ctx->k_slices_ok = 0;
  return r;
}
int32_t unet_conv3x3_bnfold_bwd_data_enc_tail(unet_ctx* ctx, const float* dy, const float* w, const float* bnp, const double* bn_bwd_sums, double count, const float* x, int32_t ldx,
                                              const float* enc_bnp, const double* enc_sums, double enc_count, const float* skip_k1, const float* dy_pooled, float rate, uint64_t seed,
                                              float* dx, float* wt_ws, float* coef, int32_t n, int32_t h, int32_t wd, int32_t c, int32_t algo, void* stream) {
  if (!ctx || !dy || !w || !bnp || !bn_bwd_sums || !x || !enc_bnp || !enc_sums || !dy_pooled || !dx || !wt_ws || !coef || n < 1 || !(count >= 1) || !(enc_count >= 1) || !(rate >= 0) || rate >= 1)
    UNET_FAIL(ctx, UNET_E_ARG, "conv3x3_bnfold_bwd_data_enc_tail: bad args");
  if (c < 32 || (c % 32) || (h & 1) || (wd & 1) || !unet_conv3x3_bnfold_supported(algo, h, wd, 2 * c, c) || !h2_enc_tail_dgrad_selected(ctx, algo, n, h, wd, c, true))
    UNET_FAIL(ctx, UNET_E_SHAPE, "conv3x3_bnfold_bwd_data_enc_tail: h=%d w=%d c=%d (even h and w, c a multiple of 32, unet_conv3x3_bnfold_supported(2 c -> c))", h, wd, c);
  hipStream_t s = as_stream(stream);
  int32_t r = k_bn_bwd_coef(ctx, bnp, bn_bwd_sums, count, coef, 2 * c, s);
  if (!r) r = k_h2_weights(ctx, w, wt_ws, 2 * c, c, 1, s);
  if (!r) r = k_conv3x3_h2_dgrad_enc_tail(ctx, dy, wt_ws, coef, x, ldx, enc_bnp, enc_sums, enc_count, skip_k1, dy_pooled, dx, n, h, wd, c, rate, seed, s);
  return r;
}

size_t unet_conv3x3_bwd_weights_ws_bytes(int32_t n, int32_t h, int32_t wd, int32_t cin, int32_t cout) {
  if (cin == 1 && (cout % 4) == 0 && 256 % (cout / 4) == 0 && cout <= 256) return c1_wgrad_ws_bytes(cout);
  return mfma_wgrad_supported(cin, cout) ? mfma_wgrad_ws_bytes(n, h, wd, cin, cout) : 0;
}

int32_t unet_conv3x3_bwd_weights(unet_ctx* ctx, const float* x, const float* dy, float* dw, float* db, void* ws, size_t ws_bytes,
                                 int32_t n, int32_t h, int32_t wd, int32_t cin, int32_t cout, int32_t algo, void* stream) {
  if (!ctx || !x || !dy || !dw || !db || n < 1 || h < 1 || wd < 1 || cin < 1 || cout < 1) UNET_FAIL(ctx, UNET_E_ARG, "conv3x3_bwd_weights: bad args");
  return conv3x3_wgrad_dispatch(ctx, x, dy, dw, db, ws, ws_bytes, n, h, wd, cin, cout, algo, as_stream(stream));
}

int32_t unet_convT2x2_fwd(unet_ctx* ctx, const float* x, const float* w, const float* bias, float* y, int32_t ldy, int32_t n,
                          int32_t h, int32_t wd, int32_t cin, int32_t cout, int32_t algo, void* stream) {
  if (!ctx || !x || !w || !y || ldy < cout || n < 1 || h < 1 || wd < 1) UNET_FAIL(ctx, UNET_E_ARG, "convT_fwd: bad args");
  if (h2_convT_selected(ctx, algo, cin, cout)) return k_convT_h2_fwd(ctx, x, w, bias, y, ldy, n, h, wd, cin, cout, as_stream(stream));
  if (algo != UNET_ALGO_NAIVE && mfma_convT_supported(cin, cout)) return k_convT_mfma_fwd(ctx, x, w, bias, y, ldy, n, h, wd, cin, cout, as_stream(stream));
  return k_convT_naive_fwd(ctx, x, w, bias, y, ldy, n, h, wd, cin, cout, as_stream(stream));
}

int32_t unet_convT2x2_bwd_data(unet_ctx* ctx, const float* dy, int32_t lddy, const float* w, const float* relu_src, float* dx,
                               int32_t n, int32_t h, int32_t wd, int32_t cin, int32_t cout, int32_t algo, void* stream) {
  if (!ctx || !dy || !w || !dx || lddy < cout) UNET_FAIL(ctx, UNET_E_ARG, "convT_bwd_data: bad args");
  if (h2_convT_selected(ctx, algo, cin, cout)) return k_convT_h2_dgrad(ctx, dy, lddy, w, relu_src, dx, n, h, wd, cin, cout, as_stream(stream));
  if (algo != UNET_ALGO_NAIVE && mfma_convT_supported(cin, cout)) return k_convT_mfma_dgrad(ctx, dy, lddy, w, relu_src, dx, n, h, wd, cin, cout, as_stream(stream));
  return k_convT_naive_dgrad(ctx, dy, lddy, w, relu_src, dx, n, h, wd, cin, cout, as_stream(stream));
}

size_t unet_convT2x2_bwd_weights_ws_bytes(int32_t n, int32_t h, int32_t wd, int32_t cin, int32_t cout) {
  return std::max(mfma_convT_supported(cin, cout) ? mfma_convT_wgrad_ws_bytes(n, h, wd, cin, cout) : 0, h2_convT_wgrad_ws_bytes(n, h, wd, cin, cout));
}

int32_t unet_convT2x2_bwd_weights(unet_ctx* ctx, const float* x, const float* dy, int32_t lddy, float* dw, float* db, void* ws,
                                  size_t ws_bytes, int32_t n, int32_t h, int32_t wd, int32_t cin, int32_t cout, int32_t algo,
                                  void* stream) {
  if (!ctx || !x || !dy || !dw || !db || lddy < cout) UNET_FAIL(ctx, UNET_E_ARG, "convT_bwd_weights: bad args");
  const bool can = mfma_convT_supported(cin, cout) && ws && ws_bytes >= mfma_convT_wgrad_ws_bytes(n, h, wd, cin, cout);
  if (h2_convT_wgrad_selected(algo, cin, cout) && ws && ws_bytes >= h2_convT_wgrad_ws_bytes(n, h, wd, cin, cout))
    return k_convT_h2_wgrad(ctx, x, dy, lddy, dw, db, ws, ws_bytes, n, h, wd, cin, cout, as_stream(stream));
  if (algo != UNET_ALGO_NAIVE && can) return k_convT_mfma_wgrad(ctx, x, dy, lddy, dw, db, ws, ws_bytes, n, h, wd, cin, cout, as_stream(stream));
  return k_convT_naive_wgrad(ctx, x, dy, lddy, dw, db, n, h, wd, cin, cout, as_stream(stream));
}


int32_t unet_conv3x3_fwd_bf16(unet_ctx* ctx, const unet_bf16* x, const float* w, const float* bias, unet_bf16* y, int32_t n, int32_t h, int32_t wd,
                              int32_t cin, int32_t cout, int32_t act, float drop_rate, uint64_t drop_seed, void* w_ws, void* stream) {
  if (!ctx || !x || !w || !y || !w_ws || n < 1 || h < 1 || wd < 1 || act < 0 || act > 2 || drop_rate < 0 || drop_rate >= 1) UNET_FAIL(ctx, UNET_E_ARG, "conv3x3_fwd_bf16: bad args");
  return k_conv3x3_bf16_fwd(ctx, x, w, bias, nullptr, MASK_NONE, y, n, h, wd, cin, cout, act, drop_rate, drop_seed, static_cast<unet_bf16*>(w_ws), 0, as_stream(stream));
}
int32_t unet_conv3x3_first_fwd_bf16(unet_ctx* ctx, const float* x, const float* w, const float* bias, unet_bf16* y, int32_t n, int32_t h, int32_t wd,
                                    int32_t cout, int32_t act, float drop_rate, uint64_t drop_seed, void* stream) {
// ... 39 lines not shown

}

namespace {

struct Layer { std::string name; int kind; int cin, cout; };
struct TInfo { int is_state; int64_t off, count; };
struct Buf { size_t off = 0; int ld = 0, n = 0, h = 0, w = 0, c = 0; size_t chan_off = 0; int f32 = 0; };

struct Op {
  std::string name;
  std::function<int32_t(hipStream_t)> run;
  double flops = 0, bytes = 0, ms = 0;
  int64_t calls = 0;
};

}

struct unet_model {
  unet_ctx* ctx = nullptr;
  int arch = 0, in_ch = 1, N = 0, H = 0, W = 0, world = 1, algo = 0;
  int dt = UNET_DTYPE_F32;
  std::vector<Layer> layers;
  std::map<std::string, TInfo> tinfo;
  int64_t n_params = 0, n_state = 0;
  float *params = nullptr, *grads = nullptr, *adam_m = nullptr, *adam_v = nullptr, *state = nullptr;
  char* ws = nullptr; size_t ws_bytes = 0;
  const float *x = nullptr, *yt = nullptr; float* pout = nullptr; float* loss_out2 = nullptr;
  float drop_rate = 0.0f; uint64_t drop_seed = 0;
  float cw0 = 1.0f, cw1 = 1.0f;
  unet_loss_sel loss;
  size_t off_wmap = 0;
  bool weighted() const { return loss.kind == UNET_LOSS_WEIGHTED_BCE_DICE; }
  const float* wmap() const { return weighted() ? reinterpret_cast<const float*>(ws) + off_wmap : nullptr; }
  size_t off_dense_ws = 0, dense_ws_bytes = 0;
  std::map<std::string, Buf> act, grad;
  size_t ws_floats_infer = 0, ws_floats_train = 0;
  size_t off_bn_sums = 0, bn_sums_doubles = 0;
  size_t off_bn_bsums = 0;
  std::map<std::string, size_t> bn_sum_off, bn_bsum_off, bnp_off;
  size_t off_loss_sums = 0, off_loss_out = 0, off_wt = 0, off_wgrad_ws = 0; size_t wgrad_ws_bytes = 0;
  size_t off_first_tmp = 0;
  bool skip_raw = false; std::map<std::string, size_t> bn_comp_off; size_t off_tap_tmp = 0;
  std::set<std::string> pool_sums_fused;
  bool c9b_virtual = false;
  bool head_bwd_fused = false;
  size_t off_head_sums = 0; bool head_fused = false;
  std::map<std::string, size_t> sign_off;
  std::map<std::string, size_t> wprep_f, wprep_b;
  std::map<std::string, size_t> fold_off, fold_g_off, fold_c_off;
  std::map<std::string, std::pair<std::string, int>> folded_bn;
  std::map<std::string, size_t> skip_k1_off;
  std::set<std::string> enc_tail_dgrad;
  std::vector<Op> prog[3];
  std::vector<unet_sync_point> sync[3];
  struct SyncRef { int after_op, kind; bool in_ws; size_t off_bytes; int64_t count; int use_op = -1; };
  std::vector<SyncRef> syncref[3];

  float* wsf(size_t off) const { return reinterpret_cast<float*>(ws) + off; }
  double* wsd(size_t off_floats) const { return reinterpret_cast<double*>(reinterpret_cast<float*>(ws) + off_floats); }
  float* P(const std::string& n) const { auto& t = tinfo.at(n); return (t.is_state ? state : params) + t.off; }
  float* G(const std::string& n) const { auto& t = tinfo.at(n); return grads + t.off; }
  const float* A(const std::string& n) const { auto& b = act.at(n); return wsf(b.off + b.chan_off); }
  float* Aw(const std::string& n) const { auto& b = act.at(n); return wsf(b.off + b.chan_off); }
  float* D(const std::string& n) const { auto& b = grad.at(n); return wsf(b.off + b.chan_off); }
  int elem_bytes(const Buf& b) const { return (dt && !b.f32) ? 2 : 4; }
  void* bufptr(const Buf& b) const { return ws + b.off * 4 + b.chan_off * elem_bytes(b); }
  void* Av(const std::string& n) const { return bufptr(act.at(n)); }
  void* Dv(const std::string& n) const { return bufptr(grad.at(n)); }
};

namespace {

const int ENC[4] = {32, 64, 128, 256};

void assign_param_offsets(unet_model* m) {
  int64_t po = 0, so = 0;
  for (auto& l : m->layers) {
    if (l.kind == 2) {
      m->tinfo[l.name + "/gamma"] = {0, po, l.cout}; po += l.cout;
      m->tinfo[l.name + "/beta"] = {0, po, l.cout}; po += l.cout;
      m->tinfo[l.name + "/mean"] = {1, so, l.cout}; so += l.cout;
      m->tinfo[l.name + "/var"] = {1, so, l.cout}; so += l.cout;
    } else {
      int64_t kn = (l.kind == 0 ? 9 : l.kind == 1 ? 4 : 1) * (int64_t)l.cin * l.cout;
      m->tinfo[l.name + "/kernel"] = {0, po, kn}; po += kn;
      m->tinfo[l.name + "/bias"] = {0, po, l.cout}; po += l.cout;
    }
  }
  m->n_params = po; m->n_state = so;
}

void build_layers(unet_model* m) {
  auto& L = m->layers;
  int cprev = m->in_ch;
  for (int k = 1; k <= 4; ++k) {
    int c = ENC[k - 1];
    L.push_back({"c" + std::to_string(k) + "a", 0, cprev, c});
    L.push_back({"c" + std::to_string(k) + "b", 0, c, c});
    L.push_back({"bn" + std::to_string(k), 2, c, c});
    cprev = c;
  }
  L.push_back({"c5a", 0, 256, 512});
  L.push_back({"c5b", 0, 512, 512});
  cprev = 512;
  const int dec[4] = {256, 128, 64, 32};
// ... 472 lines not shown
                                        m->G("out/kernel"), m->G("out/bias"), hp, hb.c, 1, s);
      return unet_head_bwd_ex(ctx, m->A("c9b"), m->P("out/kernel"), m->pout, m->yt, m->wsd(m->off_loss_sums), (double)hp * gcount, L.kind, L.alpha, L.beta, m->wmap(), m->D("c9b"),
                           m->G("out/kernel"), m->G("out/bias"), hp, hb.c, 1, s);
    });
    std::vector<Op> DEF;
    auto flush_def = [&]() { for (auto& o : DEF) BW.push_back(std::move(o)); DEF.clear(); };
    auto conv_bwd = [&](const std::string& name, const std::string& in, int cin, int cout, bool want_dx, bool mask_in, const std::string& xraw = "", bool defer_wgrad = false) {
      const Buf ob = m->act.at(name);
      const double px = (double)ob.n * ob.h * ob.w;
      const std::string xsrc = xraw.empty() ? in : xraw;
      auto& WV = (defer_wgrad && xraw.empty()) ? DEF : BW;
      const bool hstream = name == "c9b" && m->head_bwd_fused;
      ADD_OP(WV, "conv3x3_wgrad:" + name, 2.0 * 9 * cin * cout * px, (hstream ? eb * px * cin + 8.0 * px : eb * px * (cin + cout)) + 4.0 * 9.0 * cin * cout, {
        if (dt) {
          if (in.empty()) return first_conv_wgrad_bf16(ctx, m, name, ob, cout, s);
          return k_conv3x3_bf16_wgrad(ctx, CBF(m->Av(xsrc)), CBF(m->Dv(name)), m->G(name + "/kernel"), m->G(name + "/bias"), m->wsf(m->off_wgrad_ws), m->wgrad_ws_bytes, ob.n, ob.h, ob.w,
                                      cin, cout, s);
        }
        const float* xin = xsrc.empty() ? m->x : m->A(xsrc);
        if (name == "c9b" && m->head_bwd_fused)
          return k_conv3x3_h2_wgrad_dzm(ctx, xin, m->D(name), m->P("out/kernel"), m->G(name + "/kernel"), m->G(name + "/bias"), m->wsf(m->off_wgrad_ws), m->wgrad_ws_bytes, ob.n, ob.h, ob.w, cin, s);
        return conv3x3_wgrad_dispatch(ctx, xin, m->D(name), m->G(name + "/kernel"), m->G(name + "/bias"), m->wsf(m->off_wgrad_ws), m->wgrad_ws_bytes,
                                      ob.n, ob.h, ob.w, cin, cout, algo, s);
      });
      if (!xraw.empty()) {
        const size_t go = m->fold_g_off.at(name), bo = m->bnp_off.at(in);
        const bool pg = !dt && m->fold_c_off.count(name) != 0;
        ADD_OP(BW, "wgrad_bn_fold_fix:" + name, 2.0 * 9 * cin * cout, 8.0 * 9 * cin * cout, {
          if (dt) return k_wgrad_bn_fold_fix_bf16(ctx, CBF(m->Dv(name)), ob.n, ob.h, ob.w, cin, cout, m->wsf(bo), m->wsf(bo) + cin, m->G(name + "/kernel"), m->G(name + "/bias"), m->wsf(go), s,
                                                  m->P(name + "/kernel"), m->wsf(bo) + 2 * cin, m->wsf(bo) + 3 * cin, m->wsd(m->off_bn_bsums) + m->bn_bsum_off.at(in));
          if (m->skip_raw) {
            const float* comp = m->wsf(m->bn_comp_off.at(in));
            return k_wgrad_bn_fold_fix(ctx, m->D(name), ob.n, ob.h, ob.w, cin, cout, comp, comp + cin, m->G(name + "/kernel"), m->G(name + "/bias"), m->wsf(go), s,
                                       m->P(name + "/kernel"), m->wsf(bo) + 2 * cin, m->wsf(bo) + 3 * cin, m->wsd(m->off_bn_bsums) + m->bn_bsum_off.at(in), comp + 2 * cin, comp + 3 * cin,
                                       pg ? m->G(in + "/gamma") : nullptr, pg ? m->G(in + "/beta") : nullptr);
          }
          return k_wgrad_bn_fold_fix(ctx, m->D(name), ob.n, ob.h, ob.w, cin, cout, m->wsf(bo), m->wsf(bo) + cin, m->G(name + "/kernel"), m->G(name + "/bias"), m->wsf(go), s,
                                     m->P(name + "/kernel"), m->wsf(bo) + 2 * cin, m->wsf(bo) + 3 * cin, m->wsd(m->off_bn_bsums) + m->bn_bsum_off.at(in), nullptr, nullptr,
                                     pg ? m->G(in + "/gamma") : nullptr, pg ? m->G(in + "/beta") : nullptr);
        });
      }
      if (!xraw.empty() && m->fold_c_off.count(name)) {
        const std::string bnn = in;
        const size_t so = m->bn_bsum_off.at(bnn), bo = m->bnp_off.at(bnn), co = m->fold_c_off.at(name);
        ADD_OP(BW, "bn_bwd_param_grads:" + bnn, 0, 0, {
          if (!dt) return UNET_OK;
          return unet_bn_bwd_param_grads(ctx, m->wsd(m->off_bn_bsums) + so, m->G(bnn + "/gamma"), m->G(bnn + "/beta"), cin, s);
        });
        SY.push_back({(int)BW.size() - 1, 2, true, m->off_bn_bsums * 4 + so * 8, 2 * (int64_t)cin});
        const size_t syi = SY.size() - 1;
        flush_def();
        SY[syi].use_op = (int)BW.size();
        const bool half = !dt && name.size() == 3 && m->enc_tail_dgrad.count("bn" + std::to_string(10 - (name[1] - '0'))) != 0;
        ADD_OP(BW, "conv3x3_dgrad_bn_bwd:" + name, (half ? 0.5 : 1.0) * 2.0 * 9 * cin * cout * px, half ? eb * px * (cout + cin) + 4.0 * 9.0 * (cin / 2) * cout : eb * px * (cout + 2 * cin) + 4.0 * 9.0 * cin * cout, {
          int32_t r = k_bn_bwd_coef(ctx, m->wsf(bo), m->wsd(m->off_bn_bsums) + so, px * gcount, m->wsf(co), cin, s);
          if (r) return r;
          if (half) return k_conv3x3_h2_dgrad_bn_bwd_up(ctx, m->D(name), m->wsf(m->wprep_b.at(name)), m->wsf(co), m->A(xraw), m->D(xraw), ob.n, ob.h, ob.w, cout, s);
          if (dt) return k_conv3x3_bf16_fwd(ctx, CBF(m->Dv(name)), m->P(name + "/kernel"), m->wsf(co), CBF(m->Av(xraw)), MASK_BN_BWD, WBF(m->Dv(xraw)), ob.n, ob.h, ob.w, cout, cin, ACT_NONE, 0.0f, 0,
                                            WBF(static_cast<void*>(m->wsf(m->off_wt))), 1, s, CBF(static_cast<void*>(m->wsf(m->wprep_b.at(name)))));
          const int climit = m->skip_k1_off.count("bn" + std::to_string(10 - (name[1] - '0'))) ? cin / 2 : (1 << 30);
          return k_conv3x3_h2_fwd(ctx, m->D(name), m->wsf(m->wprep_b.at(name)), m->wsf(co), m->A(xraw), MASK_BN_BWD, m->D(xraw), ob.n, ob.h, ob.w, cout, cin, ACT_NONE, 0.0f, 0, s, climit);
        });
        return;
      }
      if (want_dx && !dt && !mask_in && in.size() == 2 && in[0] == 'p' && ctx->opt_enc_bn_fused && m->wprep_b.count(name) && h2_pool_sums_selected(ctx, algo, ob.w, cout, cin)) {
        const std::string bnn = "bn" + in.substr(1);
        const size_t so = m->bn_bsum_off.at(bnn);
        m->pool_sums_fused.insert(in);
        ADD_OP(BW, "conv3x3_dgrad_pool_sums:" + name, 2.0 * 9 * cin * cout * px, eb * px * (cout + 2 * cin) + 4.0 * 9.0 * cin * cout, {
          (void)so;
          return k_conv3x3_h2_dgrad_pool_sums(ctx, m->D(name), m->wsf(m->wprep_b.at(name)), m->A(in), m->P(bnn + "/gamma"), m->P(bnn + "/beta"), m->drop_rate, m->D(in),
                                              nullptr, ob.n, ob.h, ob.w, cout, cin, s);
        });
      } else
      if (want_dx) {
        const bool bits = mask_in && m->sign_off.count(in) != 0;
        ADD_OP(BW, "conv3x3_dgrad:" + name, 2.0 * 9 * cin * cout * px, (hstream ? 8.0 * px + eb * px * (cin + (mask_in ? (bits ? cin / 32.0 : cin) : 0)) : eb * px * (cout + cin + (mask_in ? (bits ? cin / 32.0 : cin) : 0))) + 4.0 * 9.0 * cin * cout, {
          if (dt) return k_conv3x3_bf16_fwd(ctx, CBF(m->Dv(name)), m->P(name + "/kernel"), nullptr, mask_in ? CBF(m->Av(in)) : nullptr, mask_in ? MASK_RELU : MASK_NONE, WBF(m->Dv(in)), ob.n, ob.h,
                                            ob.w, cout, cin, ACT_NONE, 0.0f, 0, WBF(static_cast<void*>(m->wsf(m->off_wt))), 1, s, CBF(static_cast<void*>(m->wsf(m->wprep_b.at(name)))));
          const auto pb = m->wprep_b.find(name);
          const auto so = mask_in ? m->sign_off.find(in) : m->sign_off.end();
          if (name == "c9b" && m->head_bwd_fused)
            return k_conv3x3_h2_dgrad_dzm(ctx, m->D(name), m->wsf(pb->second), so != m->sign_off.end() ? m->wsf(so->second) : mask_in ? m->A(in) : nullptr,
                                          so != m->sign_off.end() ? MASK_RELU_BITS : mask_in ? MASK_RELU : MASK_NONE, m->D(in), ob.n, ob.h, ob.w, cin, s);
          if (so != m->sign_off.end())
            return conv3x3_fwd_dispatch(ctx, m->D(name), m->P(name + "/kernel"), nullptr, m->wsf(so->second), MASK_RELU_BITS, m->D(in), ob.n, ob.h,
                                        ob.w, cout, cin, ACT_NONE, 0.0f, 0, algo, s, m->wsf(m->off_wt), 1, pb == m->wprep_b.end() ? nullptr : m->wsf(pb->second));
          return conv3x3_fwd_dispatch(ctx, m->D(name), m->P(name + "/kernel"), nullptr, mask_in ? m->A(in) : nullptr, mask_in ? MASK_RELU : MASK_NONE, m->D(in), ob.n, ob.h,
                                      ob.w, cout, cin, ACT_NONE, 0.0f, 0, algo, s, m->wsf(m->off_wt), 1, pb == m->wprep_b.end() ? nullptr : m->wsf(pb->second));
        });
      }
    };
    auto bn_bwd = [&](const std::string& name, const std::string& dyname, const std::string& xname, const std::string& dxname, int c, int mask,
                      bool stats_done) {
      const Buf gb = m->grad.at(dyname), xb = m->act.at(xname), db = m->grad.at(dxname);
      const int64_t pixels = (int64_t)xb.n * xb.h * xb.w;
      const size_t so = m->bn_bsum_off.at(name), bo = m->bnp_off.at(name);
      if (stats_done) {
        ADD_OP(BW, "bn_bwd_param_grads:" + name, 0, 0, {
          return unet_bn_bwd_param_grads(ctx, m->wsd(m->off_bn_bsums) + so, m->G(name + "/gamma"), m->G(name + "/beta"), c, s);
        });
      } else {
        ADD_OP(BW, "bn_bwd_stats:" + name, 0, 2 * eb * pixels * c, {
          int32_t r = dt ? unet_bn_bwd_stats_bf16(ctx, CBF(m->Dv(dyname)), gb.ld, CBF(m->Av(xname)), xb.ld, m->wsf(bo), m->wsd(m->off_bn_bsums) + so, pixels, c, s)
                         : unet_bn_bwd_stats(ctx, m->D(dyname), gb.ld, m->A(xname), xb.ld, m->wsf(bo), m->wsd(m->off_bn_bsums) + so, pixels, c, s);
          if (r) return r;
          return unet_bn_bwd_param_grads(ctx, m->wsd(m->off_bn_bsums) + so, m->G(name + "/gamma"), m->G(name + "/beta"), c, s);
        });
      }
      SY.push_back({(int)BW.size() - 1, 2, true, m->off_bn_bsums * 4 + so * 8, 2 * (int64_t)c});
      ADD_OP(BW, "bn_bwd_apply:" + name, 0, 3 * eb * pixels * c, {
        if (dt) return unet_bn_bwd_apply_bf16(ctx, CBF(m->Dv(dyname)), gb.ld, CBF(m->Av(xname)), xb.ld, m->wsf(bo), m->wsd(m->off_bn_bsums) + so, (double)pixels * gcount,
                                              mask ? MASK_RELU : MASK_NONE, 0.0f, 0, WBF(m->Dv(dxname)), db.ld, pixels, c, s);
        return unet_bn_bwd_apply(ctx, m->D(dyname), gb.ld, m->A(xname), xb.ld, m->wsf(bo), m->wsd(m->off_bn_bsums) + so, (double)pixels * gcount, mask ? MASK_RELU : MASK_NONE, 0.0f, 0,
                                 m->D(dxname), db.ld, pixels, c, s);
      });
    };
    auto bucket = [&](const std::string& first, const std::string& last_tensor) {
      const TInfo a = m->tinfo.at(first), b = m->tinfo.at(last_tensor);
      SY.push_back({(int)BW.size() - 1, 3, false, (size_t)a.off * 4, b.off + b.count - a.off});
    };
    if (!dt && m->skip_raw && ctx->opt_enc_bn_fused && ctx->opt_enc_tail_dgrad)
      for (int k = 1; k <= 4; ++k) {
        const std::string bnn = "bn" + std::to_string(k), dca = "c" + std::to_string(10 - k) + "a", cb = "c" + std::to_string(k) + "b";
        const Buf xb = m->act.at(bnn), cg = m->grad.at(cb);
        if (m->fold_c_off.count(dca) && m->skip_k1_off.count(bnn) && m->wprep_b.count(dca) && cg.ld == xb.c && m->act.at(dca).c == xb.c &&
            h2_enc_tail_dgrad_selected(ctx, algo, xb.n, xb.h, xb.w, xb.c, ctx->opt_enc_tail_dgrad == 2))
          m->enc_tail_dgrad.insert(bnn);
      }
    bool enc_split = false;
    const int dec[4] = {256, 128, 64, 32};
    for (int k = 9; k >= 6; --k) {
      int c = dec[k - 6]; std::string ks = std::to_string(k);
      std::string prev = (k == 6) ? "c5b" : "c" + std::to_string(k - 1) + "b";
      int cprev = (k == 6) ? 512 : dec[k - 7];
      conv_bwd("c" + ks + "b", "c" + ks + "a", c, c, true, true, "", m->fold_c_off.count("c" + ks + "a") != 0);
      conv_bwd("c" + ks + "a", "bn" + ks, 2 * c, c, true, false, m->fold_off.count("c" + ks + "a") ? "cat" + ks : "");
      flush_def();
      if (!m->fold_c_off.count("c" + ks + "a")) bn_bwd("bn" + ks, "bn" + ks, "cat" + ks, "cat" + ks, 2 * c, 0, m->fold_off.count("c" + ks + "a") != 0);
      const Buf ib = m->act.at(prev), ug = m->grad.at("u" + ks);
      const std::string un = "u" + ks;
      ADD_OP(BW, "convT_wgrad:" + un, 2.0 * 4 * cprev * c * nel(ib) / ib.c, eb * (nel(ib) + nel(ug)), {
        if (dt) return k_convT_bf16_wgrad(ctx, CBF(m->Av(prev)), CBF(m->Dv(un)), ug.ld, m->G(un + "/kernel"), m->G(un + "/bias"), m->wsf(m->off_wgrad_ws), m->wgrad_ws_bytes, ib.n, ib.h,
                                          ib.w, cprev, c, s);
        return unet_convT2x2_bwd_weights(ctx, m->A(prev), m->D(un), ug.ld, m->G(un + "/kernel"), m->G(un + "/bias"), m->wsf(m->off_wgrad_ws), m->wgrad_ws_bytes,
                                         ib.n, ib.h, ib.w, cprev, c, algo, s);
      });
      ADD_OP(BW, "convT_dgrad:" + un, 2.0 * 4 * cprev * c * nel(ib) / ib.c, eb * (2 * nel(ib) + nel(ug)), {
        if (dt) return k_convT_bf16_dgrad(ctx, CBF(m->Dv(un)), ug.ld, m->P(un + "/kernel"), CBF(m->Av(prev)), WBF(m->Dv(prev)), ib.n, ib.h, ib.w, cprev, c, WBF(static_cast<void*>(m->wsf(m->off_wt))), s);
        const auto so = m->sign_off.find(prev);
        const auto pb = m->wprep_b.find(un);
        const void* img = pb == m->wprep_b.end() ? nullptr : m->wsf(pb->second);
        if (so != m->sign_off.end()) return k_convT_h2_dgrad(ctx, m->D(un), ug.ld, m->P(un + "/kernel"), m->wsf(so->second), m->D(prev), ib.n, ib.h, ib.w, cprev, c, s, 1, img);
        if (img) return k_convT_h2_dgrad(ctx, m->D(un), ug.ld, m->P(un + "/kernel"), m->A(prev), m->D(prev), ib.n, ib.h, ib.w, cprev, c, s, 0, img);
        return unet_convT2x2_bwd_data(ctx, m->D(un), ug.ld, m->P(un + "/kernel"), m->A(prev), m->D(prev), ib.n, ib.h, ib.w, cprev, c, algo, s);
      });
      if (k == 7) bucket("u7/kernel", "out/bias");
      if (k == 6) bucket("u6/kernel", "c6b/bias");
    }
    conv_bwd("c5b", "c5a", 512, 512, true, true);
    conv_bwd("c5a", "p4", 256, 512, true, false, "", ctx->opt_enc_bn_fused != 0);
    if (!ctx->opt_enc_bn_fused) bucket("c5a/kernel", "c5b/bias");
    for (int k = 4; k >= 1; --k) {
      int c = ENC[k - 1]; std::string ks = std::to_string(k);
      const Buf xb = m->act.at("bn" + ks), gb = m->grad.at("bn" + ks);
      const std::string bnn = "bn" + ks, pn = "p" + ks;
      const size_t so = m->bn_bsum_off.at(bnn);
      if (ctx->opt_enc_bn_fused) {
        const std::string dn = "bn" + std::to_string(10 - k), cb = "c" + ks + "b";
        const size_t sod = m->bn_bsum_off.at(dn), bod = m->bnp_off.at(dn), bo = m->bnp_off.at(bnn);
        const Buf cbuf = m->act.at(cb), cg = m->grad.at(cb);
        const int64_t pixels = (int64_t)xb.n * xb.h * xb.w;
        const bool sums_done = m->pool_sums_fused.count(pn) != 0;
        ADD_OP(BW, sums_done ? "pool_bwd_skip_term:" + pn : "pool_bwd_sums:" + pn, 0, sums_done ? 0.0 : eb * 0.5 * nel(xb), {
          int32_t r = sums_done ? UNET_OK : dt ? unet_maxpool2x2_dropout_bwd_sums_bf16(ctx, CBF(m->Av(pn)), CBF(m->Dv(pn)), m->P(bnn + "/gamma"), m->P(bnn + "/beta"), m->wsd(m->off_bn_bsums) + so, xb.n, xb.h,
                                                                 xb.w, xb.c, m->drop_rate, m->drop_seed + (uint64_t)k * 0x9E3779B97F4A7C15ull, s)
                         : unet_maxpool2x2_dropout_bwd_sums(ctx, m->A(pn), m->D(pn), m->P(bnn + "/gamma"), m->P(bnn + "/beta"), m->wsd(m->off_bn_bsums) + so, xb.n, xb.h, xb.w, xb.c,
                                                            m->drop_rate, m->drop_seed + (uint64_t)k * 0x9E3779B97F4A7C15ull, s);
          if (r) return r;
          if (sums_done)
            return k_enc_tail_finish(ctx, m->wsd(m->off_bn_bsums) + so, m->wsd(m->off_bn_bsums) + sod + 3 * (size_t)c, m->wsf(bod) + 7 * (size_t)c, m->P(dn + "/gamma") + c,
                                     m->P(bnn + "/gamma"), m->G(bnn + "/gamma"), m->G(bnn + "/beta"), c, 1.0 / gcount, s);
          r = unet_bn_bwd_skip_term(ctx, m->wsd(m->off_bn_bsums) + so, m->wsd(m->off_bn_bsums) + sod + 3 * (size_t)c, m->wsf(bod) + 7 * (size_t)c, m->P(dn + "/gamma") + c,
                                    m->P(bnn + "/gamma"), c, 1.0 / gcount, s);
          if (r) return r;
          return unet_bn_bwd_param_grads(ctx, m->wsd(m->off_bn_bsums) + so, m->G(bnn + "/gamma"), m->G(bnn + "/beta"), c, s);
        });
        SY.push_back({(int)BW.size() - 1, 2, true, m->off_bn_bsums * 4 + so * 8, 2 * (int64_t)c});
        const size_t syi = SY.size() - 1;
        flush_def();
        if (k == 4) bucket("c5a/kernel", "c5b/bias");
        if (k == 2) { bucket("c3a/kernel", "bn4/beta"); enc_split = true; }
        SY[syi].use_op = (int)BW.size();
        const bool tail = m->enc_tail_dgrad.count(bnn) != 0;
        const std::string dca = "c" + std::to_string(10 - k) + "a";
        ADD_OP(BW, "bn_pool_bwd_apply:" + bnn, tail ? 2.0 * 9 * c * c * (double)pixels * unet_conv3x3_exec_ratio(algo, xb.h, xb.w, c, 2 * c) : 0.0, eb * 3.25 * nel(xb) + (tail ? 4.0 * 9.0 * c * c : 0.0), {
          if (tail)
            return k_conv3x3_h2_dgrad_enc_tail(ctx, m->D(dca), m->wsf(m->wprep_b.at(dca)), m->wsf(m->fold_c_off.at(dca)), m->A(cb), cbuf.ld, m->wsf(bo), m->wsd(m->off_bn_bsums) + so,
                                               (double)pixels * gcount, m->wsf(m->skip_k1_off.at(bnn)), m->D(pn), m->D(cb), xb.n, xb.h, xb.w, xb.c, m->drop_rate,
                                               m->drop_seed + (uint64_t)k * 0x9E3779B97F4A7C15ull, s);
          if (dt) return unet_bn_maxpool_bwd_apply_bf16(ctx, CBF(m->Av(cb)), cbuf.ld, m->wsf(bo), m->wsd(m->off_bn_bsums) + so, (double)pixels * gcount, CBF(m->Dv(bnn)), gb.ld, CBF(m->Dv(pn)),
// ... 978 lines not shown
```

Baseline: 1075 images/sec.

## Fuse ConvT data-gradient into the decoder conv3x3 BN-backward dgrad epilogue

Adds a new epilogue (EPI 6) to the 8-row conv3x3 data-gradient kernel. It takes the freshly computed upsample-branch gradient tile, splits it into scaled fp16 pairs, and runs the 2x2 transposed-conv data gradient with MFMAs. The result, masked by ReLU signs or bits, is written straight into the previous decoder block's gradient. The standalone convT_dgrad op for u9..u7 becomes a no-op when selected, which saves a full re-read of the concat gradient from global memory and a kernel launch. In exchange the kernel is larger, with extra LDS staging, syncthreads and register pressure, which may lower occupancy for the main conv.

Result: no change. 1084 images/sec (median of 6 runs) (+0.8%).

```diff
diff --git a/include/unet_hip.h b/include/unet_hip.h
--- a/include/unet_hip.h
+++ b/include/unet_hip.h
@@ -24,7 +24,8 @@
 const char* unet_last_error(const unet_ctx* ctx);
 int32_t unet_ctx_set_profiling(unet_ctx* ctx, int32_t on);
 enum { UNET_OPT_RELU_BITS = 1, UNET_OPT_BN_FOLD = 2, UNET_OPT_ENC_BN_FUSED = 3, UNET_OPT_BN_CONCAT_ANALYTIC = 4, UNET_OPT_BN_FUSE_STATS = 5, UNET_OPT_DETERMINISTIC = 6,
-       UNET_OPT_HEAD_FUSED = 7, UNET_OPT_SKIP_RAW = 8, UNET_OPT_POOL_SUMS_FUSED = 9, UNET_OPT_HEAD_BWD_FUSED = 10, UNET_OPT_CONV_PP = 13, UNET_OPT_ENC_TAIL_DGRAD = 14 };
+       UNET_OPT_HEAD_FUSED = 7, UNET_OPT_SKIP_RAW = 8, UNET_OPT_POOL_SUMS_FUSED = 9, UNET_OPT_HEAD_BWD_FUSED = 10, UNET_OPT_CONV_PP = 13, UNET_OPT_ENC_TAIL_DGRAD = 14,
+       UNET_OPT_CONVT_DGRAD_TAIL = 15 };
 int32_t unet_ctx_set_option(unet_ctx* ctx, int32_t option, int32_t value);
 int32_t unet_ctx_get_option(unet_ctx* ctx, int32_t option);
 
@@ -63,6 +64,10 @@
 int32_t unet_conv3x3_bnfold_bwd_data_enc_tail(unet_ctx*, const float* dy, const float* w, const float* bnp, const double* bn_bwd_sums, double count, const float* x, int32_t ldx,
                                               const float* enc_bnp, const double* enc_sums, double enc_count, const float* skip_k1, const float* dy_pooled, float rate,
                                               uint64_t seed, float* dx, float* wt_ws, float* coef, int32_t n, int32_t h, int32_t wd, int32_t c, int32_t algo, void* stream);
+int32_t unet_conv3x3_bnfold_bwd_data_convt_tail_supported(unet_ctx*, int32_t algo, int32_t n, int32_t h, int32_t wd, int32_t c);
+int32_t unet_conv3x3_bnfold_bwd_data_convt_tail(unet_ctx*, const float* dy, const float* w, const float* bnp, const double* bn_bwd_sums, double count, const float* x, const float* wt,
+                                                const void* relu_src, int32_t relu_bits, float* dx, float* dx_prev, float* wt_ws, float* coef, float* wt_img_ws, int32_t n, int32_t h,
+                                                int32_t wd, int32_t c, int32_t algo, void* stream);
 size_t unet_conv3x3_bwd_weights_ws_bytes(int32_t n, int32_t h, int32_t wd, int32_t cin, int32_t cout);
 int32_t unet_conv3x3_bwd_weights(unet_ctx*, const float* x, const float* dy, float* dw, float* db,
                                  void* ws, size_t ws_bytes, int32_t n, int32_t h, int32_t wd,
diff --git a/one-stop-for-covid-19-infection-and-lung-segmentation-plus-classification_amd/_lib.py b/one-stop-for-covid-19-infection-and-lung-segmentation-plus-classification_amd/_lib.py
--- a/one-stop-for-covid-19-infection-and-lung-segmentation-plus-classification_amd/_lib.py
+++ b/one-stop-for-covid-19-infection-and-lung-segmentation-plus-classification_amd/_lib.py
@@ -9,7 +9,7 @@
 COMM_HANDLE_BYTES, COMM_MAX_WORLD, COMM_MAX_DOUBLES = 64, 8, 2048
 
 ALGO_AUTO, ALGO_NAIVE, ALGO_MFMA = 0, 1, 2
-OPTIONS = {"relu_bits": 1, "bn_fold": 2, "enc_bn_fused": 3, "bn_concat_analytic": 4, "bn_fuse_stats": 5, "deterministic": 6, "head_fused": 7, "skip_raw": 8, "pool_sums_fused": 9, "head_bwd_fused": 10, "conv_pp": 13, "enc_tail_dgrad": 14}
+OPTIONS = {"relu_bits": 1, "bn_fold": 2, "enc_bn_fused": 3, "bn_concat_analytic": 4, "bn_fuse_stats": 5, "deterministic": 6, "head_fused": 7, "skip_raw": 8, "pool_sums_fused": 9, "head_bwd_fused": 10, "conv_pp": 13, "enc_tail_dgrad": 14, "convt_dgrad_tail": 15}
 ARCH_UNET, ARCH_UNETPP, ARCH_CLASSIFIER = 0, 1, 2
 LOSSES = {"bce_dice_loss": 0, "binary_crossentropy": 1, "dice_loss": 2, "tversky_loss": 3, "weighted_bce_dice_loss": 4}
 DTYPE_F32, DTYPE_BF16 = 0, 1
@@ -101,6 +101,8 @@
     "unet_conv3x3_bnfold_bwd_weights": (i32, [vp, vp, vp, vp, vp, vp, vp, vp, vp, sz, vp, i32, i32, i32, i32, i32, i32, vp]),
     "unet_conv3x3_bnfold_bwd_data": (i32, [vp, vp, vp, vp, vp, f64, vp, i32, i32, f32, u64, vp, vp, vp, i32, i32, i32, i32, i32, i32, vp]),
     "unet_conv3x3_bnfold_bwd_data_enc_tail": (i32, [vp, vp, vp, vp, vp, f64, vp, i32, vp, vp, f64, vp, vp, f32, u64, vp, vp, vp, i32, i32, i32, i32, i32, vp]),
+    "unet_conv3x3_bnfold_bwd_data_convt_tail_supported": (i32, [vp, i32, i32, i32, i32, i32]),
+    "unet_conv3x3_bnfold_bwd_data_convt_tail": (i32, [vp, vp, vp, vp, vp, f64, vp, vp, vp, i32, vp, vp, vp, vp, vp, i32, i32, i32, i32, i32, vp]),
     "unet_bn_stats_concat": (i32, [vp, vp, i32, vp, f64, vp, vp, vp, i64, i32, i32, vp]),
     "unet_bn_stats_concat_bf16": (i32, [vp, vp, i32, vp, f64, vp, vp, vp, i64, i32, i32, vp]),
     "unet_bn_finalize_train": (i32, [vp, vp, f64, vp, vp, vp, vp, vp, i32, vp]),
diff --git a/one-stop-for-covid-19-infection-and-lung-segmentation-plus-classification_amd/csrc/common.h b/one-stop-for-covid-19-infection-and-lung-segmentation-plus-classification_amd/csrc/common.h
--- a/one-stop-for-covid-19-infection-and-lung-segmentation-plus-classification_amd/csrc/common.h
+++ b/one-stop-for-covid-19-infection-and-lung-segmentation-plus-classification_amd/csrc/common.h
@@ -29,6 +29,7 @@
   int opt_head_fused = 1;
   int opt_head_bwd_fused = 1;
   int opt_enc_tail_dgrad = 1;
+  int opt_convt_dgrad_tail = 1;
   int opt_conv_pp = 1;
   int opt_deterministic = 0;
   double* bn_slots = nullptr;
@@ -278,6 +279,9 @@
 int32_t k_conv3x3_h2_dgrad_bn_bwd_up(unet_ctx*, const float* dy, const void* wimg, const float* coef, const float* x, float* dx, int n, int h, int wd, int C, hipStream_t s);
 int32_t k_conv3x3_h2_dgrad_enc_tail(unet_ctx*, const float* dy, const void* wimg, const float* coef, const float* x, int ldx, const float* enc_bnp, const double* enc_sums, double count,
                                     const float* skip_k1, const float* dy_pooled, float* dx, int n, int h, int wd, int C, float rate, uint64_t seed, hipStream_t s);
+bool h2_convt_dgrad_tail_selected(const unet_ctx* ctx, int algo, int n, int h, int wd, int C, int mode);
+int32_t k_conv3x3_h2_dgrad_bn_bwd_up_convt(unet_ctx*, const float* dy, const void* wimg, const float* coef, const float* x, float* dx, const void* timg, const void* relu, int relu_kind,
+                                           float* dx_prev, int n, int h, int wd, int C, hipStream_t s);
 bool h2_pool_sums_selected(const unet_ctx* ctx, int algo, int wd, int K, int M);
 int32_t k_conv3x3_h2_dgrad_pool_sums(unet_ctx*, const float* dy, const void* wimg, const float* pooled, const float* gamma, const float* beta, float rate, float* dx, double* sums,
                                      int n, int h, int wd, int K, int M, hipStream_t s);
diff --git a/one-stop-for-covid-19-infection-and-lung-segmentation-plus-classification_amd/csrc/kernels_conv_h2.hip b/one-stop-for-covid-19-infection-and-lung-segmentation-plus-classification_amd/csrc/kernels_conv_h2.hip
--- a/one-stop-for-covid-19-infection-and-lung-segmentation-plus-classification_amd/csrc/kernels_conv_h2.hip
+++ b/one-stop-for-covid-19-infection-and-lung-segmentation-plus-classification_amd/csrc/kernels_conv_h2.hip
@@ -124,6 +124,10 @@
   constexpr bool ETAIL = EPI == 5;
   static_assert(!ETAIL || (MODE == 0 && RW == 2 && !GEN && !SPLITK), "the encoder-tail epilogue rides on the 8-row conv3x3 data-gradient launches");
   if (ETAIL) { mask_mode = MASK_BN_BWD; act = ACT_NONE; stats = nullptr; signs = nullptr; }
+  constexpr bool CTAIL = EPI == 6;
+  constexpr bool CT_LDS = CTAIL && NB == 1;
+  static_assert(!CTAIL || (MODE == 0 && RW == 2 && !GEN && !SPLITK), "the ConvT data-gradient tail rides on the 8-row conv3x3 data-gradient launches");
+  if (CTAIL) { mask_mode = MASK_BN_BWD; act = ACT_NONE; stats = nullptr; signs = nullptr; }
   static_assert(!VDY || (MODE == 0 && NB == 1 && RW == 2 && !GEN), "the virtual head gradient feeds the 32-channel data-gradient launch");
   static_assert(!HEAD || (MODE == 0 && NB == 1 && RW == 2 && !GEN), "the fused head rides on the 32-channel forward kernel");
   static_assert(!POOLS || (MODE == 0 && !GEN), "the pooled sums ride on a plain conv3x3 data-gradient launch");
@@ -605,6 +609,9 @@
     H2_STAMP(8);
     return;
   }
+  float ct_mx = 0.f;
+  int ct_base = wave * (RW * 32 * OUT_PS);
+  if (CT_LDS) asm volatile("" : "+v"(ct_base));
 #pragma unroll
   for (int nb = 0; nb < NB; ++nb) {
     const int mb0 = (g * NB + nb) * 32, mb = mb0 + hi * 16;
@@ -621,8 +628,15 @@
 #pragma unroll
     for (int r = 0; r < RW; ++r) {
       const int py = y0 + wave * RW + r;
-      if (py >= H) continue;
+      if (py >= H) {
+        if constexpr (CTAIL && !CT_LDS) {
+#pragma unroll
+          for (int i = 0; i < 16; ++i) acc[r][nb][i] = 0.f;
+        }
+        continue;
+      }
       const bool live = px_ < W && mb < M;
+      char* const s_row = CT_LDS ? smem + ct_base + r * (32 * OUT_PS) : s_out;
       long long o;
       if (MODE == 1) o = (((long long)n * 2 * H + 2 * py + (ab >> 1)) * (2 * W) + 2 * px_ + (ab & 1)) * ldy + oc;
       else o = (((long long)n * H + py) * W + px_) * ldy + mb;
@@ -648,12 +662,12 @@
       } else if (want_m && !POOLS) {
         if (MPF) {
 #pragma unroll
-          for (int j = 0; j < 4; ++j) *reinterpret_cast<float4*>(s_out + out_cell(j * 8 + (lane >> 3), lane & 7)) = mpre[MPF ? nb : 0][MPF ? r : 0][j];
+          for (int j = 0; j < 4; ++j) *reinterpret_cast<float4*>(s_row + out_cell(j * 8 + (lane >> 3), lane & 7)) = mpre[MPF ? nb : 0][MPF ? r : 0][j];
         }
 #pragma unroll
         for (int q = 0; q < 4; ++q) {
           float4 m4;
-          if (MPF) m4 = *reinterpret_cast<const float4*>(s_out + out_cell(l31, hi * 4 + q));
+          if (MPF) m4 = *reinterpret_cast<const float4*>(s_row + out_cell(l31, hi * 4 + q));
           else m4 = (live && mb0 < mask_climit) ? *reinterpret_cast<const float4*>(mask + (((long long)n * H + py) * W + px_) * ldm + (mb - c_off) + q * 4) : make_float4(0.f, 0.f, 0.f, 0.f);
           mv[q * 4] = m4.x; mv[q * 4 + 1] = m4.y; mv[q * 4 + 2] = m4.z; mv[q * 4 + 3] = m4.w;
         }
@@ -724,19 +738,23 @@
           }
         }
       }
+      if constexpr (CTAIL) {
+#pragma unroll
+        for (int i = 0; i < 16; ++i) { if (CT_LDS) break; const float t = live ? v[i] : 0.f; acc[r][nb][i] = t; ct_mx = fmaxf(ct_mx, fabsf(t)); }
+      }
 #pragma unroll
       for (int q = 0; q < 4; ++q)
-        *reinterpret_cast<float4*>(s_out + out_cell(l31, hi * 4 + q)) = make_float4(v[q * 4], v[q * 4 + 1], v[q * 4 + 2], v[q * 4 + 3]);
+        *reinterpret_cast<float4*>(s_row + out_cell(l31, hi * 4 + q)) = make_float4(v[q * 4], v[q * 4 + 1], v[q * 4 + 2], v[q * 4 + 3]);
       float4 t4s[4];
       if (!GEN) {
 #pragma unroll
-        for (int j = 0; j < 4; ++j) t4s[j] = *reinterpret_cast<const float4*>(s_out + out_cell(j * 8 + (lane >> 3), lane & 7));
+        for (int j = 0; j < 4; ++j) t4s[j] = *reinterpret_cast<const float4*>(s_row + out_cell(j * 8 + (lane >> 3), lane & 7));
         asm volatile("" :: "v"(t4s[0].x), "v"(t4s[1].x), "v"(t4s[2].x), "v"(t4s[3].x));
       }
 #pragma unroll
       for (int j = 0; j < 4; ++j) {
         const int pj = j * 8 + (lane >> 3), cj = lane & 7, pxj = x0 + pj;
-        const float4 t4 = GEN ? *reinterpret_cast<const float4*>(s_out + out_cell(pj, cj)) : t4s[j];
+        const float4 t4 = GEN ? *reinterpret_cast<const float4*>(s_row + out_cell(pj, cj)) : t4s[j];
         long long oj;
         if (MODE == 1) oj = (((long long)n * 2 * H + 2 * py + (ab >> 1)) * (2 * W) + 2 * pxj + (ab & 1)) * ldy + (oc - hi * 16);
         else oj = (((long long)n * H + py) * W + pxj) * ldy + (mb - hi * 16);
@@ -784,6 +802,136 @@
       }
     }
   }
+  if constexpr (CTAIL) {
+    constexpr int NOB = 2 * NB, CAB = 2 * 64 * 16 + 64, CPL = 4 * CAB;
+    constexpr int CWP = 4 * NOB * 128, CWL = CWP / 256;
+    static_assert(2 * CPL <= IN_BYTES && CWP * 16 <= W_LDS && CWL <= WL, "the ConvT tail's pieces go through the conv's own patch and slab regions");
+    __builtin_amdgcn_sched_barrier(0);
+    int tid = threadIdx.x;
+    asm volatile("" : "+v"(tid));
+    const int lane = tid & 63, l31 = lane & 31, hi = lane >> 5, px_ = x0 + l31;
+    char* const s_out = smem + wave * (32 * OUT_PS);
+    const int Hh = H >> 1, Wh = W >> 1, pp = wave >> 1, ob0 = (wave & 1) * NB;
+    const float tw_unscale = *hd.w;
+    const __amdgpu_buffer_rsrc_t rs_t = __builtin_amdgcn_make_buffer_rsrc(const_cast<unet_bf16*>(reinterpret_cast<const unet_bf16*>(hd.w) + H2_HEADER / 2), 0, (K >> 4) * CWP * 16, 0x00020000);
+    auto ct_w_loads = [&](int piece) __attribute__((always_inline)) {
+#pragma unroll
+      for (int k = 0; k < CWL; ++k) {
+        const int idx = tid + k * 256, abi = idx / (NOB * 128), within = idx - abi * (NOB * 128);
+        wreg[k] = __builtin_amdgcn_raw_buffer_load_b128(rs_t, (abi * (K >> 4) * NOB * 128 + within) * 16, piece * NOB * 2048, 0);
+      }
+    };
+    ct_w_loads(0);
+    unsigned ct_raw[NB];
+#pragma unroll
+    for (int nb = 0; nb < NB; ++nb) {
+      ct_raw[nb] = 0u;
+      const int j = l31 >> 3, gi = (y0 >> 1) + 2 * pp + (j >> 1), cx = (x0 >> 4) + (j & 1);
+      if (hd.aux == 2.0f && hi == 0 && gi < Hh && cx * 8 < Wh)
+        ct_raw[nb] = reinterpret_cast<const unsigned*>(hd.t)[((((long long)n * Hh + gi) * (Wh >> 3) + cx) * (M >> 5) + ob0 + nb) * 8 + (lane & 7)];
+    }
+    if constexpr (CT_LDS) {
+      static_assert(!CT_LDS || 4 * RW * 32 * OUT_PS <= IN_BYTES + W_LDS, "a staging row per image row of the tile");
+#pragma unroll
+      for (int r = 0; r < RW; ++r) {
+        const bool ok = y0 + wave * RW + r < H && px_ < W;
+#pragma unroll
+        for (int q = 0; q < 4; ++q) {
+          const float4 g4 = *reinterpret_cast<const float4*>(smem + (wave * RW + r) * (32 * OUT_PS) + out_cell(l31, hi * 4 + q));
+          acc[r][0][q * 4] = ok ? g4.x : 0.f; acc[r][0][q * 4 + 1] = ok ? g4.y : 0.f; acc[r][0][q * 4 + 2] = ok ? g4.z : 0.f; acc[r][0][q * 4 + 3] = ok ? g4.w : 0.f;
+          ct_mx = fmaxf(fmaxf(ct_mx, fmaxf(fabsf(acc[r][0][q * 4]), fabsf(acc[r][0][q * 4 + 1]))), fmaxf(fabsf(acc[r][0][q * 4 + 2]), fabsf(acc[r][0][q * 4 + 3])));
+        }
+      }
+    }
+    ct_mx = wave_max_nonneg(ct_mx);
+    if (lane == 0) s_amax[wave] = ct_mx;
+    __syncthreads();
+    const float bm = fmaxf(fmaxf(s_amax[0], s_amax[1]), fmaxf(s_amax[2], s_amax[3]));
+    const int eb2 = __builtin_amdgcn_readfirstlane((int)((__float_as_uint(bm) >> 23) & 0xFF));
+    const int e2 = (eb2 >= 11 && eb2 - 127 + 120 >= 15) ? scale_exp_for(eb2) : 120;
+    const float sc2 = pow2f(e2);
+    f32x16 acc2[NB];
+#pragma unroll
+    for (int nb = 0; nb < NB; ++nb)
+#pragma unroll
+      for (int i = 0; i < 16; ++i) acc2[nb][i] = 0.0f;
+#pragma unroll
+    for (int piece = 0; piece < 2 * NB; ++piece) {
+      if (hi == (piece & 1)) {
+#pragma unroll
+        for (int r = 0; r < RW; ++r) {
+          unsigned hh[8], mm[8];
+#pragma unroll
+          for (int q = 0; q < 8; ++q) split2_scaled(acc[r][piece >> 1][2 * q], acc[r][piece >> 1][2 * q + 1], sc2, hh[q], mm[q]);
+          char* p = s_in + (r * 2 + (l31 & 1)) * CAB + (wave * 16 + (l31 >> 1)) * 16;
+          *reinterpret_cast<uint4*>(p) = make_uint4(hh[0], hh[1], hh[2], hh[3]); *reinterpret_cast<uint4*>(p + 1024) = make_uint4(hh[4], hh[5], hh[6], hh[7]);
+          *reinterpret_cast<uint4*>(p + CPL) = make_uint4(mm[0], mm[1], mm[2], mm[3]); *reinterpret_cast<uint4*>(p + CPL + 1024) = make_uint4(mm[4], mm[5], mm[6], mm[7]);
+        }
+      }
+#pragma unroll
+      for (int k = 0; k < CWL; ++k) *reinterpret_cast<unet_u32x4*>(s_w + (tid + k * 256) * 16) = wreg[k];
+      __syncthreads();
+      if (piece + 1 < 2 * NB) ct_w_loads(piece + 1);
+      __builtin_amdgcn_s_setprio(2);
+#pragma unroll
+      for (int ab = 0; ab < 4; ++ab) {
+        f16x8 px[2], wf[NB][2];
+#pragma unroll
+        for (int p = 0; p < 2; ++p) px[p] = lds_frag(s_in + p * CPL + ab * CAB + (hi * 64 + pp * 32 + l31) * 16);
+#pragma unroll
+        for (int nb = 0; nb < NB; ++nb)
+#pragma unroll
+          for (int p = 0; p < 2; ++p) wf[nb][p] = lds_frag(s_w + ((((ab * NOB + ob0 + nb) * 2 + p) * 2 + hi) * 512 + l31 * 16));
+#pragma unroll
+        for (int pr = 0; pr < 3; ++pr) {
+          constexpr int PW[3] = {0, 1, 0}, PX[3] = {1, 0, 0};
+#pragma unroll
+          for (int nb = 0; nb < NB; ++nb) acc2[nb] = __builtin_amdgcn_mfma_f32_32x32x16_f16(wf[nb][PW[pr]], px[PX[pr]], acc2[nb], 0, 0, 0);
+        }
+      }
+      __builtin_amdgcn_s_setprio(0);
+      __syncthreads();
+    }
+    const float unscale2 = pow2f(-e2) * tw_unscale;
+    unsigned ct_bits[NB];
+#pragma unroll
+    for (int nb = 0; nb < NB; ++nb) {
+      ct_bits[nb] = hd.aux == 2.0f ? 0u : 0xFFFFu;
+      if (hd.aux == 2.0f) {
+#pragma unroll
+        for (int jk = 0; jk < 16; ++jk) ct_bits[nb] |= (((unsigned)__shfl((int)ct_raw[nb], jk * 2 + hi) >> l31) & 1u) << jk;
+      }
+    }
+#pragma unroll
+    for (int nb = 0; nb < NB; ++nb) {
+#pragma unroll
+      for (int q = 0; q < 4; ++q)
+        *reinterpret_cast<float4*>(s_out + out_cell(l31, hi * 4 + q)) = make_float4(acc2[nb][q * 4] * unscale2, acc2[nb][q * 4 + 1] * unscale2, acc2[nb][q * 4 + 2] * unscale2, acc2[nb][q * 4 + 3] * unscale2);
+      float4 t4s[4];
+#pragma unroll
+      for (int j = 0; j < 4; ++j) t4s[j] = *reinterpret_cast<const float4*>(s_out + out_cell(j * 8 + (lane >> 3), lane & 7));
+      asm volatile("" :: "v"(t4s[0].x), "v"(t4s[1].x), "v"(t4s[2].x), "v"(t4s[3].x));
+#pragma unroll
+      for (int j = 0; j < 4; ++j) {
+        const int gi = (y0 >> 1) + 2 * pp + (j >> 1), gj = (x0 >> 1) + (j & 1) * 8 + (lane >> 3);
+        if (gi < Hh && gj < Wh) {
+          float4 t4 = t4s[j];
+          const long long o = (((long long)n * Hh + gi) * Wh + gj) * M + (ob0 + nb) * 32 + (lane & 7) * 4;
+          if (hd.aux == 1.0f) {
+            const float4 m4 = *reinterpret_cast<const float4*>(hd.t + o);
+            t4.x = m4.x > 0.f ? t4.x : 0.f; t4.y = m4.y > 0.f ? t4.y : 0.f; t4.z = m4.z > 0.f ? t4.z : 0.f; t4.w = m4.w > 0.f ? t4.w : 0.f;
+          } else {
+            const unsigned b = ct_bits[nb] >> (j * 4);
+            t4.x = (b & 1u) ? t4.x : 0.f; t4.y = (b & 2u) ? t4.y : 0.f; t4.z = (b & 4u) ? t4.z : 0.f; t4.w = (b & 8u) ? t4.w : 0.f;
+          }
+          float* const q = hd.p + o;
+          __builtin_nontemporal_store(t4.x, q); __builtin_nontemporal_store(t4.y, q + 1); __builtin_nontemporal_store(t4.z, q + 2); __builtin_nontemporal_store(t4.w, q + 3);
+        }
+      }
+    }
+    H2_STAMP(8);
+    return;
+  }
   H2_STAMP(12);
   if (MODE != 2 && stats) {
     __syncthreads();
@@ -814,7 +962,7 @@
                   int splits = 1, int g0 = 0, int ng = 0, int ldm = 0, int c_off = 0) {
   constexpr int T = MODE == 0 ? 9 : 1, KS = MODE == 0 ? 1 : 2;
   if (img_nb == 0) img_nb = NB;
-  if (img_nb != NB && !(MODE != 2 && NB == 1 && (img_nb == 2 || img_nb == 4) && (M % (32 * img_nb)) == 0 && (EPI == 0 || EPI == 5))) UNET_FAIL(ctx, UNET_E_ARG, "conv h2: image of %d blocks per group on a %d-block launch", img_nb, NB);
+  if (img_nb != NB && !(MODE != 2 && NB == 1 && (img_nb == 2 || img_nb == 4) && (M % (32 * img_nb)) == 0 && (EPI == 0 || EPI == 5 || EPI == 6))) UNET_FAIL(ctx, UNET_E_ARG, "conv h2: image of %d blocks per group on a %d-block launch", img_nb, NB);
   constexpr int TH = 4 * RW;
   constexpr int NPIX = MODE == 0 ? (TH + 2) * 34 : TH * 32;
   constexpr size_t smem = (size_t)2 * KS * 2 * (NPIX * 16 + (MODE == 0 ? 0 : 64)) + (NB != 1 || MODE != 0 ? (size_t)((KS * T * NB * 2 * 2 * 32 + 255) / 256) * 256 * 16 : (size_t)KS * T * NB * 2 * 2 * 32 * 16) + 16 + 3 * NB * 32 * 4;
@@ -870,6 +1018,11 @@
     r = go(conv_h2_kernel<MODE, NB, RW, false, WPS, EPI>);
   } else if (EPI == 5) {
     if (!mask || !bias || !hd.w || !hd.b || !hd.slots || act != ACT_NONE || (h & 1) || (wd & 1) || rate < 0.0f || rate >= 1.0f) UNET_FAIL(ctx, UNET_E_ARG, "conv h2 + encoder tail: a plain data-gradient launch over an even image only");
+    r = go(conv_h2_kernel<MODE, NB, RW, false, WPS, EPI>);
+  } else if (EPI == 6) {
+    if (!mask || !bias || !hd.w || !hd.p || (hd.aux != 0.0f && !hd.t) || act != ACT_NONE || rate != 0.0f || (h & 1) || (wd & 1) || M != 2 * K || K != 32 * NB || g0 != 0 || groups != 1 ||
+        (hd.aux == 2.0f && ((wd >> 1) & 7)))
+      UNET_FAIL(ctx, UNET_E_ARG, "conv h2 + ConvT data-gradient tail: the up-half launch of C = %d channels over an even image only", 32 * NB);
     r = go(conv_h2_kernel<MODE, NB, RW, false, WPS, EPI>);
   } else if (EPI == 3) {
     if (gen || K != 32 || ldx != 2 || act != ACT_NONE || mask_mode == MASK_POOL_SUMS) UNET_FAIL(ctx, UNET_E_ARG, "conv h2 behind the head's {dz, mask} stream: a plain 32-channel data-gradient launch only");
@@ -1055,6 +1208,24 @@
     return launch_h2<0, 2, 4, 2>(ctx, dy, C, img, coef, x, MASK_BN_BWD, dx, M, n, h, wd, C, M, ACT_NONE, 0.0f, 0, s, 1 << 30, h2_head_args(), 0, 1, 0, C / 64);
   return launch_h2<0, 2, 2, 2>(ctx, dy, C, img, coef, x, MASK_BN_BWD, dx, M, n, h, wd, C, M, ACT_NONE, 0.0f, 0, s, 1 << 30, h2_head_args(), 0, 1, 0, C / 64);
 }
+bool h2_convt_dgrad_tail_selected(const unet_ctx* ctx, int algo, int n, int h, int wd, int C, int mode) {
+  if (!ctx || mode < 1 || (C != 32 && C != 64) || n < 1 || h < 2 || wd < 2 || (h & 1) || (wd & 1) || !h2_conv3x3_selected(algo, C, 2 * C) || (long long)h * wd * 2 * C * 4 >= (1LL << 30)) return false;
+  if (C == 64 && h <= 128 && (long long)((wd + 31) / 32) * ((h + 15) / 16) * n >= 512) return false;
+  if (mode >= 2) return true;
+  int spc; const long long wgs = h2_half_wgs(n, h, wd, C, true, &spc);
+  return wgs >= 2LL * spc * ctx->num_cu;
+}
+int32_t k_conv3x3_h2_dgrad_bn_bwd_up_convt(unet_ctx* ctx, const float* dy, const void* wimg, const float* coef, const float* x, float* dx, const void* timg, const void* relu, int relu_kind,
+                                           float* dx_prev, int n, int h, int wd, int C, hipStream_t s) {
+  if (!dy || !wimg || !coef || !x || !dx || !timg || !dx_prev || relu_kind < 0 || relu_kind > 2 || (relu_kind && !relu)) UNET_FAIL(ctx, UNET_E_ARG, "conv3x3 dgrad, up half + ConvT tail: bad args");
+  if (!h2_convt_dgrad_tail_selected(ctx, UNET_ALGO_AUTO, n, h, wd, C, 2) || (relu_kind == 2 && ((wd >> 1) & 7)))
+    UNET_FAIL(ctx, UNET_E_SHAPE, "conv3x3 dgrad, up half + ConvT tail: h=%d w=%d C=%d (C 32 or 64, even h and w, 8-row tiles; sign bits: w / 2 a multiple of 8)", h, wd, C);
+  h2_head_args hd; hd.w = static_cast<const float*>(timg); hd.t = static_cast<const float*>(relu); hd.aux = (float)relu_kind; hd.p = dx_prev;
+  const unet_bf16* img = static_cast<const unet_bf16*>(wimg);
+  const int M = 2 * C;
+  if (C == 32) return launch_h2<0, 1, 2, 4, 6>(ctx, dy, C, img, coef, x, MASK_BN_BWD, dx, M, n, h, wd, C, M, ACT_NONE, 0.0f, 0, s, 1 << 30, hd, 2, 1, 0, 1);
+  return launch_h2<0, 2, 2, 2, 6>(ctx, dy, C, img, coef, x, MASK_BN_BWD, dx, M, n, h, wd, C, M, ACT_NONE, 0.0f, 0, s, 1 << 30, hd, 0, 1, 0, 1);
+}
 int32_t k_conv3x3_h2_dgrad_enc_tail(unet_ctx* ctx, const float* dy, const void* wimg, const float* coef, const float* x, int ldx, const float* enc_bnp, const double* enc_sums, double count,
                                     const float* skip_k1, const float* dy_pooled, float* dx, int n, int h, int wd, int C, float rate, uint64_t seed, hipStream_t s) {
   if (!dy || !wimg || !coef || !x || !enc_bnp || !enc_sums || !dy_pooled || !dx || C < 32 || (C % 32) || ldx < C || (ldx & 3) || (h & 1) || (wd & 1) || !(count >= 1) || rate < 0.f || rate >= 1.f)
diff --git a/one-stop-for-covid-19-infection-and-lung-segmentation-plus-classification_amd/csrc/model.hip b/one-stop-for-covid-19-infection-and-lung-segmentation-plus-classification_amd/csrc/model.hip
--- a/one-stop-for-covid-19-infection-and-lung-segmentation-plus-classification_amd/csrc/model.hip
+++ b/one-stop-for-covid-19-infection-and-lung-segmentation-plus-classification_amd/csrc/model.hip
@@ -59,13 +59,14 @@
     case UNET_OPT_HEAD_BWD_FUSED: return &ctx->opt_head_bwd_fused;
     case UNET_OPT_CONV_PP: return &ctx->opt_conv_pp;
     case UNET_OPT_ENC_TAIL_DGRAD: return &ctx->opt_enc_tail_dgrad;
+    case UNET_OPT_CONVT_DGRAD_TAIL: return &ctx->opt_convt_dgrad_tail;
     default: return nullptr;
   }
 }
 int32_t unet_ctx_set_option(unet_ctx* ctx, int32_t option, int32_t value) {
   if (!ctx) return UNET_E_ARG;
   int* p = ctx_option(ctx, option);
-  const int hi = option == UNET_OPT_BN_FOLD ? 3 : (option == UNET_OPT_CONV_PP || option == UNET_OPT_ENC_TAIL_DGRAD) ? 2 : 1;
+  const int hi = option == UNET_OPT_BN_FOLD ? 3 : (option == UNET_OPT_CONV_PP || option == UNET_OPT_ENC_TAIL_DGRAD || option == UNET_OPT_CONVT_DGRAD_TAIL) ? 2 : 1;
   if (!p || value < 0 || value > hi) UNET_FAIL(ctx, UNET_E_ARG, "ctx_set_option: option %d value %d", option, value);
   *p = value;
   return UNET_OK;
@@ -350,6 +351,24 @@
   int32_t r = k_bn_bwd_coef(ctx, bnp, bn_bwd_sums, count, coef, 2 * c, s);
   if (!r) r = k_h2_weights(ctx, w, wt_ws, 2 * c, c, 1, s);
   if (!r) r = k_conv3x3_h2_dgrad_enc_tail(ctx, dy, wt_ws, coef, x, ldx, enc_bnp, enc_sums, enc_count, skip_k1, dy_pooled, dx, n, h, wd, c, rate, seed, s);
+  return r;
+}
+int32_t unet_conv3x3_bnfold_bwd_data_convt_tail_supported(unet_ctx* ctx, int32_t algo, int32_t n, int32_t h, int32_t wd, int32_t c) {
+  return ctx && unet_conv3x3_bnfold_supported(algo, h, wd, 2 * c, c) && h2_convt_dgrad_tail_selected(ctx, algo, n, h, wd, c, ctx->opt_convt_dgrad_tail) ? 1 : 0;
+}
+int32_t unet_conv3x3_bnfold_bwd_data_convt_tail(unet_ctx* ctx, const float* dy, const float* w, const float* bnp, const double* bn_bwd_sums, double count, const float* x, const float* wt,
+                                                const void* relu_src, int32_t relu_bits, float* dx, float* dx_prev, float* wt_ws, float* coef, float* wt_img_ws, int32_t n, int32_t h,
+                                                int32_t wd, int32_t c, int32_t algo, void* stream) {
+  if (!ctx || !dy || !w || !bnp || !bn_bwd_sums || !x || !wt || !dx || !dx_prev || !wt_ws || !coef || !wt_img_ws || n < 1 || !(count >= 1) || relu_bits < 0 || relu_bits > 1)
+    UNET_FAIL(ctx, UNET_E_ARG, "conv3x3_bnfold_bwd_data_convt_tail: bad args");
+  if ((h & 1) || (wd & 1) || !unet_conv3x3_bnfold_supported(algo, h, wd, 2 * c, c) || !h2_convt_dgrad_tail_selected(ctx, algo, n, h, wd, c, 2) || (relu_src && relu_bits && ((wd >> 1) & 7)))
+    UNET_FAIL(ctx, UNET_E_SHAPE, "conv3x3_bnfold_bwd_data_convt_tail: h=%d w=%d c=%d (even h and w, c 32 or 64 on the 8-row tiles, sign bits: w / 2 a multiple of 8)", h, wd, c);
+  hipStream_t s = as_stream(stream);
+  int32_t r = k_bn_bwd_coef(ctx, bnp, bn_bwd_sums, count, coef, 2 * c, s);
+  if (!r) r = k_h2_weights(ctx, w, wt_ws, 2 * c, c, 1, s);
+  const float* ws[1] = {wt}; void* is[1] = {wt_img_ws}; const int tcin = 2 * c, tcout = c, kind = 3;
+  if (!r) r = k_h2_prep_multi(ctx, ws, nullptr, is, &tcin, &tcout, &kind, 1, s);
+  if (!r) r = k_conv3x3_h2_dgrad_bn_bwd_up_convt(ctx, dy, wt_ws, coef, x, dx, wt_img_ws, relu_src, relu_src ? (relu_bits ? 2 : 1) : 0, dx_prev, n, h, wd, c, s);
   return r;
 }
 
@@ -495,6 +514,7 @@
   std::map<std::string, std::pair<std::string, int>> folded_bn;
   std::map<std::string, size_t> skip_k1_off;
   std::set<std::string> enc_tail_dgrad;
+  std::set<std::string> convt_dgrad_tail;
   std::vector<Op> prog[3];
   std::vector<unet_sync_point> sync[3];
   struct SyncRef { int after_op, kind; bool in_ws; size_t off_bytes; int64_t count; int use_op = -1; };
@@ -1073,9 +1093,18 @@
         flush_def();
         SY[syi].use_op = (int)BW.size();
         const bool half = !dt && name.size() == 3 && m->enc_tail_dgrad.count("bn" + std::to_string(10 - (name[1] - '0'))) != 0;
-        ADD_OP(BW, "conv3x3_dgrad_bn_bwd:" + name, (half ? 0.5 : 1.0) * 2.0 * 9 * cin * cout * px, half ? eb * px * (cout + cin) + 4.0 * 9.0 * (cin / 2) * cout : eb * px * (cout + 2 * cin) + 4.0 * 9.0 * cin * cout, {
+        const std::string tun = name.size() == 3 ? "u" + name.substr(1, 1) : std::string(), tprev = name.size() == 3 ? "c" + std::to_string(name[1] - '0' - 1) + "b" : std::string();
+        const bool ctail = half && m->convt_dgrad_tail.count(tun) != 0;
+        ADD_OP(BW, "conv3x3_dgrad_bn_bwd:" + name, (half ? 0.5 : 1.0) * 2.0 * 9 * cin * cout * px + (ctail ? 2.0 * cin * cout * px : 0.0),
+               (half ? eb * px * (cout + cin) + 4.0 * 9.0 * (cin / 2) * cout : eb * px * (cout + 2 * cin) + 4.0 * 9.0 * cin * cout) + (ctail ? eb * px * cin / 4.0 * (1.0 + 1.0 / 32.0) : 0.0), {
           int32_t r = k_bn_bwd_coef(ctx, m->wsf(bo), m->wsd(m->off_bn_bsums) + so, px * gcount, m->wsf(co), cin, s);
           if (r) return r;
+          if (ctail) {
+            const auto sg = m->sign_off.find(tprev);
+            return k_conv3x3_h2_dgrad_bn_bwd_up_convt(ctx, m->D(name), m->wsf(m->wprep_b.at(name)), m->wsf(co), m->A(xraw), m->D(xraw), m->wsf(m->wprep_b.at(tun)),
+                                                      sg != m->sign_off.end() ? static_cast<const void*>(m->wsf(sg->second)) : static_cast<const void*>(m->A(tprev)), sg != m->sign_off.end() ? 2 : 1,
+                                                      m->D(tprev), ob.n, ob.h, ob.w, cout, s);
+          }
           if (half) return k_conv3x3_h2_dgrad_bn_bwd_up(ctx, m->D(name), m->wsf(m->wprep_b.at(name)), m->wsf(co), m->A(xraw), m->D(xraw), ob.n, ob.h, ob.w, cout, s);
           if (dt) return k_conv3x3_bf16_fwd(ctx, CBF(m->Dv(name)), m->P(name + "/kernel"), m->wsf(co), CBF(m->Av(xraw)), MASK_BN_BWD, WBF(m->Dv(xraw)), ob.n, ob.h, ob.w, cout, cin, ACT_NONE, 0.0f, 0,
                                             WBF(static_cast<void*>(m->wsf(m->off_wt))), 1, s, CBF(static_cast<void*>(m->wsf(m->wprep_b.at(name)))));
@@ -1149,6 +1178,16 @@
             h2_enc_tail_dgrad_selected(ctx, algo, xb.n, xb.h, xb.w, xb.c, ctx->opt_enc_tail_dgrad == 2))
           m->enc_tail_dgrad.insert(bnn);
       }
+    if (!dt && ctx->opt_convt_dgrad_tail)
+      for (int k = 9; k >= 7; --k) {
+        const std::string un = "u" + std::to_string(k), ca = "c" + std::to_string(k) + "a", prev = "c" + std::to_string(k - 1) + "b";
+        if (!m->enc_tail_dgrad.count("bn" + std::to_string(10 - k)) || !m->wprep_b.count(un) || !m->wprep_b.count(ca) || !m->fold_c_off.count(ca)) continue;
+        const Buf ob = m->act.at(ca), ib = m->act.at(prev), ug = m->grad.at(un), cg = m->grad.at("cat" + std::to_string(k));
+        const bool bits = m->sign_off.count(prev) != 0;
+        if (ib.c == 2 * ob.c && 2 * ib.h == ob.h && 2 * ib.w == ob.w && ug.off == cg.off && ug.chan_off == 0 && ug.ld == 2 * ob.c && (!bits || (ib.w & 7) == 0) && h2_convT_selected(ctx, algo, ib.c, ob.c) &&
+            h2_convt_dgrad_tail_selected(ctx, algo, ob.n, ob.h, ob.w, ob.c, ctx->opt_convt_dgrad_tail))
+          m->convt_dgrad_tail.insert(un);
+      }
     bool enc_split = false;
     const int dec[4] = {256, 128, 64, 32};
     for (int k = 9; k >= 6; --k) {
@@ -1167,7 +1206,9 @@
         return unet_convT2x2_bwd_weights(ctx, m->A(prev), m->D(un), ug.ld, m->G(un + "/kernel"), m->G(un + "/bias"), m->wsf(m->off_wgrad_ws), m->wgrad_ws_bytes,
                                          ib.n, ib.h, ib.w, cprev, c, algo, s);
       });
-      ADD_OP(BW, "convT_dgrad:" + un, 2.0 * 4 * cprev * c * nel(ib) / ib.c, eb * (2 * nel(ib) + nel(ug)), {
+      const bool ctail = m->convt_dgrad_tail.count(un) != 0;
+      ADD_OP(BW, "convT_dgrad:" + un, ctail ? 0.0 : 2.0 * 4 * cprev * c * nel(ib) / ib.c, ctail ? 0.0 : eb * (2 * nel(ib) + nel(ug)), {
+        if (ctail) return UNET_OK;
         if (dt) return k_convT_bf16_dgrad(ctx, CBF(m->Dv(un)), ug.ld, m->P(un + "/kernel"), CBF(m->Av(prev)), WBF(m->Dv(prev)), ib.n, ib.h, ib.w, cprev, c, WBF(static_cast<void*>(m->wsf(m->off_wt))), s);
         const auto so = m->sign_off.find(prev);
         const auto pb = m->wprep_b.find(un);
```
